# yupbank/tensorframes

Measured on AMD Instinct MI355X. Metric: rows/sec map_blocks MatMul on 10M-row DF at 1/2/4/8 MI355X, higher is better.
Workload: dtype fp32; 1 GPU; model=map_blocks relu(matmul(x[?,512], W[512,512])) float32, global_batch=10000000, seq_len=512, parallelism=dp1, partitions=4, rows=10000000

## Files before the change

csrc/bindings.cpp:

```cpp
#include <torch/extension.h>

#include <unordered_map>
#include <ATen/hip/HIPContext.h>
#include <c10/hip/HIPGuard.h>

#include "comm/comm.h"
#include "ir/graph.h"
#include "kernels/kernels.h"
#include "runtime/device_pool.h"
#include "runtime/executor.h"
#include "runtime/fusion.h"
#include "runtime/jit.h"
#include "runtime/jpeg_decode.h"
#include <rocprofiler-sdk-roctx/roctx.h>

namespace py = pybind11;
using namespace tfa;

namespace tfa {
void register_packer(py::module& m);
void register_pyencode(py::module& m);
}

namespace {

py::object shape_to_py(const Shape& s) {
  if (s.unknown_rank) return py::none();
  py::list l;
  for (auto d : s.dims) l.append(d);
  return l;
}

Shape shape_from_py(const py::object& o) {
  if (o.is_none()) return Shape::unknown();
  std::vector<int64_t> d;
  for (auto v : o) d.push_back(v.is_none() ? -1 : v.cast<int64_t>());
  return Shape(d);
}

const char* row_name(RowClass r) {
  switch (r) {
    case RowClass::CONST: return "const";
    case RowClass::ROW: return "row";
    default: return "mixed";
  }
}

std::map<std::string, TensorInfo> infos_from_py(const py::dict& d) {
  std::map<std::string, TensorInfo> m;
  for (auto kv : d) {
    auto t = kv.second.cast<py::tuple>();
    TensorInfo ti;
    ti.dtype = static_cast<DType>(t[0].cast<int>());
    ti.shape = shape_from_py(t[1]);
    m[kv.first.cast<std::string>()] = ti;
  }
  return m;
}

py::list infos_to_py(const std::vector<TensorInfo>& v) {
  py::list l;
  for (auto& ti : v) {
    py::dict d;
    d["dtype"] = static_cast<int>(ti.dtype);
    d["shape"] = shape_to_py(ti.shape);
    d["row"] = row_name(ti.row);
    d["const"] = ti.value.has_value();
    l.append(d);
  }
  return l;
}

py::dict infer_all(const std::string& bytes) {
  auto g = Graph::from_bytes(bytes);
  std::vector<TensorRef> all;
  for (size_t i = 0; i < g->nodes().size(); ++i) all.push_back({static_cast<int>(i), 0});
  auto order = g->closure(all);
  Graph::Infos infos = g->infer(order, {}, false);
  py::dict out;
  for (size_t i = 0; i < g->nodes().size(); ++i) out[py::str(g->node(i).name)] = infos_to_py(infos[i]);
  return out;
}

template <typename F, typename S>
at::Tensor key_image_typed(const at::Tensor& keys, at::ScalarType st) {
  at::Tensor out = pool_empty({keys.size(0)}, keys.options().dtype(st));
  const F* in = keys.data_ptr<F>();
  S* o = out.data_ptr<S>();
  const S flip = std::numeric_limits<S>::max();
  for (int64_t i = 0; i < keys.size(0); ++i) {
    F v = in[i];
    if (v != v) v = std::numeric_limits<F>::quiet_NaN();
    if (v == F(0)) v = F(0);
    S b;
    std::memcpy(&b, &v, sizeof(b));
    o[i] = b < 0 ? S(b ^ flip) : b;
  }
  return out;
}

template <typename F, typename S>
at::Tensor key_from_image_typed(const at::Tensor& img, at::ScalarType st) {
  at::Tensor out = pool_empty({img.size(0)}, img.options().dtype(st));
  const S* in = img.data_ptr<S>();
  F* o = out.data_ptr<F>();
  const S flip = std::numeric_limits<S>::max();
  for (int64_t i = 0; i < img.size(0); ++i) {
    S b = in[i] < 0 ? S(in[i] ^ flip) : in[i];
    std::memcpy(&o[i], &b, sizeof(b));
  }
  return out;
}

at::Tensor host_key_image(const at::Tensor& keys) {
  return keys.scalar_type() == at::kDouble ? key_image_typed<double, int64_t>(keys, at::kLong)
                                           : key_image_typed<float, int32_t>(keys, at::kInt);
}

at::Tensor host_key_from_image(const at::Tensor& img, at::ScalarType st) {
  return st == at::kDouble ? key_from_image_typed<double, int64_t>(img, st) : key_from_image_typed<float, int32_t>(img, st);
}

template <size_t N>
int name_index(const char* const (&names)[N], const std::string& s) {
  for (size_t i = 0; i < N; ++i)
    if (s == names[i]) return static_cast<int>(i);
  return -1;
}

void require_stat_type(at::ScalarType st, const std::string& subject, const char* object) {
  if (st != at::kFloat && st != at::kDouble && st != at::kLong && st != at::kInt && st != at::kShort &&
      st != at::kChar && st != at::kByte)
    throw py::type_error(str_cat(subject, c10::toString(st), object, ", which is not supported (uint8, int8, int16, "
                                 "int32, int64, float32 or float64)"));
}

void stat_column(const char* what, const at::Tensor& t, const std::string& which) {
  if (!t.is_cuda()) throw py::value_error(str_cat(what, ": ", which, " must be a device tensor"));
  if (t.dim() != 1) throw py::value_error(str_cat(what, ": ", which, " must be 1-D (one scalar per row)"));
  require_stat_type(t.scalar_type(), str_cat(what, ": ", which, " is "), "");
  if (!t.is_contiguous())
    throw py::value_error(str_cat(what, ": ", which, " is not contiguous; make it contiguous first"));
}

void stat_column_like(const char* what, const at::Tensor& t, const std::string& which, const char* ref,
                      const at::Device& dev, int64_t n, DType* dtype, const void** ptr) {
  stat_column(what, t, which);
  if (t.device() != dev) throw py::value_error(str_cat(what, ": ", which, " is not on ", ref, "'s device"));
  if (t.size(0) != n) throw py::value_error(str_cat(what, ": ", which, " has ", t.size(0), " rows, ", ref, " ", n));
  *dtype = from_scalar_type(t.scalar_type());
  *ptr = t.data_ptr();
}

k::StatCols stat_cols_from(const char* what, const std::vector<at::Tensor>& cols) {
  if (cols.empty() || cols.size() > static_cast<size_t>(k::kMaxPackCols))
    throw py::value_error(str_cat(what, ": 1..", k::kMaxPackCols, " columns per call, got ", cols.size()));
  k::StatCols sc;
  sc.n = static_cast<int>(cols.size());
  stat_column(what, cols[0], "column 0");
  for (size_t c = 0; c < cols.size(); ++c)
    stat_column_like(what, cols[c], str_cat("column ", c), "the first column", cols[0].device(), cols[0].size(0),
                     &sc.dtype[c], &sc.ptr[c]);
  return sc;
}

}

namespace tfa {
namespace k {
void set_conv_smallc(int on);
void set_conv_direct(int on);
}
void set_pool_conv_fusion(bool on);
}

static thread_local int g_sort_last_passes = 0;

PYBIND11_MODULE(TORCH_EXTENSION_NAME, m) {
  m.doc() = "tensorframes_amd native runtime (GraphDef executor + HIP/CDNA4 kernels)";

  py::register_exception<GraphError>(m, "GraphError", PyExc_ValueError);
  py::register_exception<comm::CollectiveError>(m, "CollectiveError", PyExc_RuntimeError);

  py::class_<Graph, std::shared_ptr<Graph>>(m, "Graph")
      .def(py::init([](py::bytes b) { return Graph::from_bytes(std::string(b)); }))
      .def("structure_key", [](const Graph& g) { return g.structure_key(); },
           "hash of the graph without its parameter constants' payloads (Graph::structure_key)")
      .def("parameter_consts",
           [](const Graph& g) {
             std::vector<std::string> v;
             const auto& p = g.parameter_consts();
             for (size_t i = 0; i < p.size(); ++i)
               if (p[i]) v.push_back(g.node(static_cast<int>(i)).name);
             return v;
           })
      .def("node_names",
           [](const Graph& g) {
             std::vector<std::string> v;
             for (auto& n : g.nodes()) v.push_back(n.name);
             return v;
           })
      .def("node_ops",
           [](const Graph& g) {
             std::vector<std::string> v;
             for (auto& n : g.nodes()) v.push_back(n.op);
             return v;
           })
      .def("node_inputs",
           [](const Graph& g, const std::string& name) {
             int i = g.find(name);
             TFA_CHECK(i >= 0, "no node named '", name, "'");
             return g.def().nodes[i].inputs;
           })
      .def("placeholders",
           [](const Graph& g) {
             std::vector<std::string> v;
             for (int i : g.placeholders()) v.push_back(g.node(i).name);
             return v;
           })
      .def("zero_input_nodes",
           [](const Graph& g) {
             std::vector<std::string> v;
             for (auto& n : g.nodes())
               if (n.inputs.empty() && n.control.empty()) v.push_back(n.name);
             return v;
           })
      .def("has_node", [](const Graph& g, const std::string& n) { return g.find(n) >= 0; })
      .def("node_attr_scalars",
           [](const Graph& g, const std::string& name) {
             int i = g.find(name);
             TFA_CHECK(i >= 0, "no node named '", name, "'");
             py::dict d;
             for (auto& kv : g.def().nodes[i].attr) {
               const AttrValue& a = kv.second;
               switch (a.kind) {
                 case AttrValue::I: d[py::str(kv.first)] = a.i; break;
                 case AttrValue::F: d[py::str(kv.first)] = a.f; break;
                 case AttrValue::B: d[py::str(kv.first)] = a.b; break;
                 case AttrValue::TYPE: d[py::str(kv.first)] = static_cast<int>(a.type); break;
                 case AttrValue::S: d[py::str(kv.first)] = py::bytes(a.s); break;
                 default: break;
               }
             }
             return d;
           })
      .def("const_strings",
           [](const Graph& g, const std::string& name) {
             int i = g.find(name);
             TFA_CHECK(i >= 0, "no node named '", name, "'");
             const NodeDef& nd = g.def().nodes[i];
             py::list l;
             const AttrValue* v = nd.find_attr("value");
             if (nd.op == "Const" && v && v->tensor && v->tensor->dtype == DType::STRING)
               for (auto& str : v->tensor->strings) l.append(py::bytes(str));
             return l;
           })
      .def("serialize", [](const Graph& g) { return py::bytes(serialize_graphdef(g.def())); })
      .def("__len__", [](const Graph& g) { return g.nodes().size(); });

  py::class_<Program, std::shared_ptr<Program>>(m, "Program")
      .def(py::init([](std::shared_ptr<Graph> g, std::vector<std::string> fetches,
                       std::vector<std::string> feeds) {
             return std::make_shared<Program>(g, fetches, feeds);
           }),
           py::arg("graph"), py::arg("fetches"), py::arg("feeds"))
      .def_property_readonly("fetch_names", &Program::fetch_names)
      .def_property_readonly("feed_names", &Program::feed_names)
      .def("row_separable",
           [](const Program& p, py::dict hints) { return p.row_separable(infos_from_py(hints)); })
      .def("rebind", &Program::rebind, py::arg("values"), py::call_guard<py::gil_scoped_release>(),
           "a program with new parameter-constant payloads that takes over this one's plans")
      .def("adopt", &Program::adopt, py::arg("old"), py::call_guard<py::gil_scoped_release>(),
           "take over the plans of a structurally equal program (see executor.h)")
      .def("monoids",
           [](const Program& p) {
             py::list l;
             for (auto& mi : p.monoids()) l.append(py::make_tuple(mi.fetch, mi.placeholder, mi.op));
             return l;
           })
      .def("run", &Program::run, py::call_guard<py::gil_scoped_release>())
      .def("run_concurrent", &Program::run_concurrent, py::arg("inputs_list"), py::arg("max_streams") = 4,
           py::call_guard<py::gil_scoped_release>(),
           "independent runs over several input sets on one GPU, forked onto engine side streams and joined "
           "back into the caller's stream")
      .def("run_chunked", &Program::run_chunked, py::arg("seg_inputs"), py::arg("seg_outputs"),
           py::arg("chunk_rows"), py::arg("device"), py::arg("depth") = 3, py::arg("wait") = true,
           py::call_guard<py::gil_scoped_release>())
      .def("release_pipeline", &Program::release_pipeline, py::call_guard<py::gil_scoped_release>(),
           "drain and free the persistent chunk pipeline (after a deferred run_chunked sequence)")
      .def("run_chunked_reduce", &Program::run_chunked_reduce, py::arg("seg_inputs"), py::arg("chunk_rows"),
           py::arg("device"), py::arg("depth") = 3, py::call_guard<py::gil_scoped_release>())
      .def("describe", &Program::describe_plan, py::arg("inputs"), py::arg("as_gpu") = false)
      .def("fused_sources", &Program::fused_sources)
      .def("reset_stats", &Program::reset_stats)
      .def("stats", [](const Program& p) {
        ExecStats s = p.stats();
        py::dict d;
        d["runs"] = s.runs;
        d["kernels"] = s.kernels;
        d["plans_built"] = s.plans_built;
        d["plans_adopted"] = s.plans_adopted;
        d["h2d_bytes"] = s.h2d_bytes;
        d["d2h_bytes"] = s.d2h_bytes;
        d["chunks"] = s.chunks;
        d["wall_ms"] = s.wall_ms;
        d["plan_ms"] = s.plan_ms;
        d["exec_ms"] = s.exec_ms;
        d["h2d_ms"] = s.h2d_ms;
        d["compute_ms"] = s.compute_ms;
        d["d2h_ms"] = s.d2h_ms;
        d["graphs_captured"] = s.graphs_captured;
        d["graph_replays"] = s.graph_replays;
        d["graph_failures"] = s.graph_failures;
        d["graphs_declined"] = s.graphs_declined;
        d["graph_busy"] = s.graph_busy;
        return d;
      });

  m.def("analyze_fetches",
        [](std::shared_ptr<Graph> g, std::vector<std::string> fetches, std::vector<std::string> feeds,
           py::dict hints) {
          Program p(g, fetches, feeds);
          Graph::Infos infos = p.analyze(infos_from_py(hints));
          py::dict out;
          auto info_of = [&](const std::string& f) -> py::object {
            TensorRef r = g->resolve(f);
            TFA_CHECK(r.index < static_cast<int>(infos[r.node].size()), "tensor '", f,
                      "' does not exist (node has ", infos[r.node].size(), " outputs)");
            py::list l = infos_to_py({infos[r.node][r.index]});
            return py::object(l[0]);
          };
          for (auto& f : fetches) out[py::str(f)] = info_of(f);
          for (auto& f : feeds) out[py::str(f)] = info_of(f);
          return out;
        });
  m.def("infer_fed",
        [](std::shared_ptr<Graph> g, std::vector<std::string> fetches, std::vector<std::string> feeds,
           py::dict hints) {
          Program p(g, fetches, feeds);
          Graph::Infos infos = p.analyze(infos_from_py(hints));
          py::dict out;
          for (size_t i = 0; i < infos.size(); ++i)
            if (!infos[i].empty()) out[py::str(g->node(static_cast<int>(i)).name)] = infos_to_py(infos[i]);
          return out;
        });
  m.def("infer_all", &infer_all);
  m.def("light_graphdef", [](py::bytes b, int64_t max_elems) {
    GraphDef g = parse_graphdef(std::string(b));
    for (auto& nd : g.nodes) {
      if (nd.op != "Const") continue;
      const AttrValue* v = nd.find_attr("value");
      if (!v || !v->tensor || v->tensor->num_elements() <= max_elems) continue;
      AttrValue dt;
      dt.kind = AttrValue::TYPE;
      dt.type = v->tensor->dtype;
      AttrValue shp;
      shp.kind = AttrValue::SHAPE;
      shp.shape = v->tensor->shape;
      nd.op = "Placeholder";
      nd.attr.clear();
      nd.attr["dtype"] = dt;
      nd.attr["shape"] = shp;
    }
    return py::bytes(serialize_graphdef(g));
  });
  m.def("patch_graphdef", [](py::bytes orig, py::bytes patch) {
    GraphDef g = parse_graphdef(std::string(orig));
    GraphDef p = parse_graphdef(std::string(patch));
    std::unordered_map<std::string, size_t> at;
    for (size_t i = 0; i < g.nodes.size(); ++i) at[g.nodes[i].name] = i;
    for (auto& nd : p.nodes) {
      auto it = at.find(nd.name);
      if (it != at.end()) g.nodes[it->second] = nd;
      else g.nodes.push_back(nd);
    }
    return py::bytes(serialize_graphdef(g));
  });
  m.def("registered_ops", [] { return OpRegistry::get().names(); });
  m.def("set_f32_precision", [](int mode) { k::set_f32_precision(mode); });
  m.def("factorize", [](const at::Tensor& keys0) {
    TFA_CHECK(keys0.dim() == 1, "factorize: keys must be 1-D");
    at::Tensor keys = keys0.contiguous();
    const int64_t n = keys.size(0);
    if (!keys.is_cuda()) {
      const bool fl = keys.scalar_type() == at::kFloat || keys.scalar_type() == at::kDouble;
      at::Tensor img = fl ? host_key_image(keys) : keys;
      auto r = at::_unique2(img, true, true, false);
      at::Tensor uniq = fl ? host_key_from_image(std::get<0>(r), keys.scalar_type()) : std::get<0>(r);
      return py::make_tuple(std::get<1>(r).to(at::kLong), uniq);
    }
    c10::hip::HIPGuard guard(keys.device().index());
    auto opts = keys.options();
    if (n == 0) return py::make_tuple(pool_empty({0}, opts.dtype(at::kLong)), pool_empty({0}, opts));
    hipStream_t s = c10::hip::getCurrentHIPStream(keys.device().index()).stream();
    const DType dt = from_scalar_type(keys.scalar_type());
    const size_t wsb = k::factorize_workspace_bytes(dt, n);
    at::Tensor ws = pool_empty({static_cast<int64_t>(wsb)}, opts.dtype(at::kByte));
    at::Tensor ids = pool_empty({n}, opts.dtype(at::kLong));
    at::Tensor uniq = pool_empty({n}, opts);
    int64_t nseg = 0;
    {
      py::gil_scoped_release nogil;
      nseg = k::factorize(dt, keys.data_ptr(), n, ids.data_ptr<int64_t>(), uniq.data_ptr(), ws.data_ptr(), wsb, s);
    }
    return py::make_tuple(ids, uniq.narrow(0, 0, nseg));
  }, "keys [n] -> (group id per row int64, distinct keys ascending)");
  m.def("string_words", [](const at::Tensor& offsets, const at::Tensor& data, int64_t W) {
    TFA_CHECK(offsets.scalar_type() == at::kLong && offsets.dim() == 1 && offsets.size(0) >= 1,
              "string_words: offsets must be int64[n+1]");
    TFA_CHECK(data.scalar_type() == at::kByte && data.dim() == 1, "string_words: data must be uint8[bytes]");
    TFA_CHECK(W >= 1 && W <= 4096, "string_words: 1..4096 words");
    TFA_CHECK(offsets.device() == data.device(), "string_words: offsets and data on different devices");
    const int64_t n = offsets.size(0) - 1;
    at::Tensor oc = offsets.contiguous(), dc = data.contiguous();
    if (!oc.is_cuda()) {
      at::Tensor out = at::empty({W + 1, n}, oc.options());
      const int64_t* o = oc.data_ptr<int64_t>();
      const uint8_t* d = dc.data_ptr<uint8_t>();
      int64_t* y = out.data_ptr<int64_t>();
      for (int64_t i = 0; i < n; ++i) {
        const int64_t a = o[i], len = o[i + 1] - a;
        for (int64_t w = 0; w < W; ++w) {
          uint64_t v = 0;
          for (int b = 0; b < 8; ++b) {
            const int64_t j = w * 8 + b;
            v |= static_cast<uint64_t>(j < len ? d[a + j] : 0) << (56 - 8 * b);
          }
          y[w * n + i] = static_cast<int64_t>(v ^ 0x8000000000000000ull);
        }
        y[W * n + i] = len;
      }
      return out;
    }
    c10::hip::HIPGuard guard(oc.device().index());
    at::Tensor out = pool_empty({W + 1, n}, oc.options());
    k::string_words(oc.data_ptr<int64_t>(), dc.data_ptr<uint8_t>(), n, static_cast<int>(W), out.data_ptr<int64_t>(),
                    c10::hip::getCurrentHIPStream(oc.device().index()).stream());
    return out;
  }, py::arg("offsets"), py::arg("data"), py::arg("words"),
        "string keys -> [words + 1, n] int64: big-endian 8-byte words (sign-flipped) + byte length; signed order "
        "of the columns = lexicographic order of the strings");
  m.def("string_key_hash", [](const at::Tensor& offsets, const at::Tensor& data) {
    TFA_CHECK(offsets.scalar_type() == at::kLong && offsets.dim() == 1 && offsets.size(0) >= 1,
              "string_key_hash: offsets must be int64[n+1]");
    TFA_CHECK(data.scalar_type() == at::kByte && data.dim() == 1, "string_key_hash: data must be uint8[bytes]");
    TFA_CHECK(offsets.device() == data.device(), "string_key_hash: offsets and data on different devices");
    const int64_t n = offsets.size(0) - 1;
    at::Tensor oc = offsets.contiguous(), dc = data.contiguous();
    if (!oc.is_cuda()) {
      at::Tensor out = at::empty({2, n}, oc.options());
      const int64_t* o = oc.data_ptr<int64_t>();
      const uint8_t* d = dc.data_ptr<uint8_t>();
      int64_t* y = out.data_ptr<int64_t>();
      for (int64_t i = 0; i < n; ++i) {
        const int64_t a = o[i], len = o[i + 1] - a;
        uint64_t v = 0;
        for (int b = 0; b < 8; ++b) v |= static_cast<uint64_t>(b < len ? d[a + b] : 0) << (56 - 8 * b);
        y[i] = static_cast<int64_t>(v ^ 0x8000000000000000ull);
        y[n + i] = len > 8 ? static_cast<int64_t>(k::string_key_hash_host(d + a, len) + 9) : len;
      }
      return out;
    }
    c10::hip::HIPGuard guard(oc.device().index());
    at::Tensor out = pool_empty({2, n}, oc.options());
    k::string_key_hash(oc.data_ptr<int64_t>(), dc.data_ptr<uint8_t>(), n, out.data_ptr<int64_t>(),
                   c10::hip::getCurrentHIPStream(oc.device().index()).stream());
    return out;
  }, py::arg("offsets"), py::arg("data"),
        "bounded-width string keys -> [2, n] int64: sign-flipped big-endian word 0, tag = length for keys of "
        "<= 8 bytes, else 9 + a 62-bit hash of the whole key");
  m.def("string_verify", [](const at::Tensor& offsets, const at::Tensor& data, const at::Tensor& ids,
                            const at::Tensor& rep) {
    TFA_CHECK(offsets.scalar_type() == at::kLong && ids.scalar_type() == at::kLong && rep.scalar_type() == at::kLong,
              "string_verify: int64 offsets / ids / representatives");
    const int64_t n = offsets.size(0) - 1;
    TFA_CHECK(ids.dim() == 1 && ids.size(0) == n, "string_verify: one id per string");
    TFA_CHECK(offsets.device() == data.device() && ids.device() == data.device() && rep.device() == data.device(),
              "string_verify: tensors on different devices");
    at::Tensor oc = offsets.contiguous(), dc = data.contiguous(), ic = ids.contiguous(), rc = rep.contiguous();
    if (!oc.is_cuda()) {
      const int64_t* o = oc.data_ptr<int64_t>();
      const uint8_t* d = dc.data_ptr<uint8_t>();
      const int64_t* id = ic.data_ptr<int64_t>();
      const int64_t* r = rc.data_ptr<int64_t>();
      for (int64_t i = 0; i < n; ++i) {
        const int64_t a = o[i], len = o[i + 1] - a, q = r[id[i]];
        if (len <= 8 || q == i) continue;
        if (o[q + 1] - o[q] != len || std::memcmp(d + a, d + o[q], len) != 0) return false;
      }
      return true;
    }
    c10::hip::HIPGuard guard(oc.device().index());
    hipStream_t st = c10::hip::getCurrentHIPStream(oc.device().index()).stream();
    at::Tensor flag = pool_empty({1}, oc.options().dtype(at::kInt));
    TFA_CHECK(hipMemsetAsync(flag.data_ptr(), 0, sizeof(int), st) == hipSuccess, "string_verify: memset failed");
    k::string_verify(oc.data_ptr<int64_t>(), dc.data_ptr<uint8_t>(), ic.data_ptr<int64_t>(), rc.data_ptr<int64_t>(), n,
                     flag.data_ptr<int>(), st);
    return flag.item<int>() == 0;
  }, "True when every string equals its group representative's (no hash collision)");
  m.def("gather_strings", [](const at::Tensor& offsets, const at::Tensor& data, const at::Tensor& idx) {
    TFA_CHECK(offsets.is_cuda() && data.is_cuda() && idx.is_cuda() && offsets.scalar_type() == at::kLong &&
                  idx.scalar_type() == at::kLong && data.scalar_type() == at::kByte,
              "gather_strings: device int64 offsets / idx and uint8 data expected");
    c10::hip::HIPGuard guard(data.device().index());
    hipStream_t st = c10::hip::getCurrentHIPStream(data.device().index()).stream();
    at::Tensor oc = offsets.contiguous(), ic = idx.contiguous(), dc = data.contiguous();
    const int64_t n = ic.numel();
    at::Tensor lens = pool_empty({std::max<int64_t>(n, 1)}, oc.options());
    k::string_lens(oc.data_ptr<int64_t>(), ic.data_ptr<int64_t>(), n, lens.data_ptr<int64_t>(), st);
    at::Tensor new_offs = at::empty({n + 1}, at::TensorOptions().dtype(at::kLong));
    int64_t* no = new_offs.data_ptr<int64_t>();
    no[0] = 0;
    if (n) {
      std::vector<int64_t> lh(n);
      TFA_CHECK(hipMemcpyAsync(lh.data(), lens.data_ptr(), n * sizeof(int64_t), hipMemcpyDeviceToHost, st) == hipSuccess &&
                    hipStreamSynchronize(st) == hipSuccess, "gather_strings: length copy failed");
      for (int64_t g = 0; g < n; ++g) no[g + 1] = no[g] + lh[g];
    }
    at::Tensor out = pool_empty({std::max<int64_t>(no[n], 1)}, dc.options());
    if (n) {
      at::Tensor dno = pool_empty({n + 1}, oc.options());
      TFA_CHECK(hipMemcpyAsync(dno.data_ptr(), no, (n + 1) * sizeof(int64_t), hipMemcpyHostToDevice, st) == hipSuccess,
                "gather_strings: offset copy failed");
      k::gather_bytes(dc.data_ptr<uint8_t>(), oc.data_ptr<int64_t>(), ic.data_ptr<int64_t>(), dno.data_ptr<int64_t>(), n,
                      out.data_ptr<uint8_t>(), st);
      TFA_CHECK(hipStreamSynchronize(st) == hipSuccess, "gather_strings: gather failed");
    }
    return py::make_tuple(new_offs, out.narrow(0, 0, no[n]));
  }, "rows idx of a device string column -> (host int64 offsets [n+1], device uint8 bytes)");
  m.def("key_dest", [](const std::vector<at::Tensor>& keys, int64_t world) {
    TFA_CHECK(!keys.empty() && keys[0].is_cuda(), "key_dest: device key columns expected");
    c10::hip::HIPGuard guard(keys[0].device().index());
    const int64_t n = keys[0].size(0);
    hipStream_t s = c10::hip::getCurrentHIPStream(keys[0].device().index()).stream();
    at::Tensor h = pool_empty({n}, keys[0].options().dtype(at::kLong));
    for (size_t i = 0; i < keys.size(); ++i) {
      at::Tensor kc = keys[i].contiguous();
      TFA_CHECK(kc.dim() == 1 && kc.size(0) == n, "key_dest: key columns must be 1-D of equal length");
      k::key_hash(from_scalar_type(kc.scalar_type()), kc.data_ptr(), n,
                  reinterpret_cast<uint64_t*>(h.data_ptr<int64_t>()), i > 0, s);
    }
    at::Tensor dest = pool_empty({n}, h.options());
    k::hash_mod(reinterpret_cast<const uint64_t*>(h.data_ptr<int64_t>()), n, world, dest.data_ptr<int64_t>(), s);
    return dest;
  }, "destination rank of every row: hash(keys) % world (same on every rank)");
  m.def("group_representatives", [](const at::Tensor& ids, int64_t nseg) {
    TFA_CHECK(ids.is_cuda() && ids.scalar_type() == at::kLong && ids.dim() == 1, "group_representatives: device int64 ids");
    c10::hip::HIPGuard guard(ids.device().index());
    at::Tensor rep = pool_empty({nseg}, ids.options());
    k::group_representatives(ids.contiguous().data_ptr<int64_t>(), ids.size(0), nseg, rep.data_ptr<int64_t>(),
                             c10::hip::getCurrentHIPStream(ids.device().index()).stream());
    return rep;
  }, "the last row index of every group (device), as the host path's rep[ids] = arange(n)");
  m.def("partition_rows", [](const at::Tensor& dest0, int64_t world) {
    TFA_CHECK(dest0.is_cuda() && dest0.scalar_type() == at::kLong && dest0.dim() == 1, "partition_rows: device int64 dest");
    c10::hip::HIPGuard guard(dest0.device().index());
    at::Tensor dest = dest0.contiguous();
    const int64_t n = dest.size(0);
    hipStream_t s = c10::hip::getCurrentHIPStream(dest.device().index()).stream();
    const size_t wsb = k::partition_workspace_bytes(n);
    at::Tensor ws = pool_empty({static_cast<int64_t>(wsb)}, dest.options().dtype(at::kByte));
    at::Tensor perm = pool_empty({n}, dest.options());
    at::Tensor counts = pool_empty({world}, dest.options());
    k::partition_rows(dest.data_ptr<int64_t>(), n, world, perm.data_ptr<int64_t>(), counts.data_ptr<int64_t>(),
                      ws.data_ptr(), wsb, s);
    return py::make_tuple(perm, counts);
  }, "rows ordered by destination rank (stable) + rows per destination (device)");
  m.def("segment_csr", [](const at::Tensor& ids0, int64_t nseg) {
    TFA_CHECK(ids0.is_cuda() && ids0.dim() == 1 && (ids0.scalar_type() == at::kLong || ids0.scalar_type() == at::kInt),
              "segment_csr: device int ids");
    c10::hip::HIPGuard guard(ids0.device().index());
    at::Tensor ids = ids0.contiguous();
    const int64_t n = ids.size(0);
    hipStream_t s = c10::hip::getCurrentHIPStream(ids.device().index()).stream();
    at::Tensor perm = pool_empty({n}, ids.options().dtype(at::kLong));
    at::Tensor off = pool_empty({nseg + 1}, ids.options().dtype(at::kLong));
    const size_t wsb = k::segment_csr_workspace_bytes(n, nseg);
    at::Tensor ws = pool_empty({static_cast<int64_t>(wsb)}, ids.options().dtype(at::kByte));
    k::segment_csr(from_scalar_type(ids.scalar_type()), ids.data_ptr(), n, nseg, perm.data_ptr<int64_t>(),
                   off.data_ptr<int64_t>(), ws.data_ptr(), wsb, s);
    return py::make_tuple(perm, off);
  }, "ids [n] in [0, nseg) -> (rows ordered by segment, stable; CSR offsets [nseg + 1]) on the device");
  m.def("segment_rows", [](const at::Tensor& perm, const at::Tensor& offs, int64_t size) {
    TFA_CHECK(perm.is_cuda() && offs.is_cuda() && perm.scalar_type() == at::kLong && offs.scalar_type() == at::kLong,
              "segment_rows: device int64 tensors");
    c10::hip::HIPGuard guard(perm.device().index());
    const int64_t G = offs.size(0);
    at::Tensor idx = pool_empty({G * size}, perm.options());
    k::segment_rows(perm.contiguous().data_ptr<int64_t>(), offs.contiguous().data_ptr<int64_t>(), G, size,
                    idx.data_ptr<int64_t>(), c10::hip::getCurrentHIPStream(perm.device().index()).stream());
    return idx;
  }, "row ids of G equal-size segments: perm[offs[g] + j] for j < size -> [G * size]");
  m.def("scatter_rows", [](at::Tensor dst, const at::Tensor& idx, const at::Tensor& src0) {
    TFA_CHECK(dst.is_cuda() && idx.is_cuda() && src0.is_cuda() && idx.scalar_type() == at::kLong,
              "scatter_rows: device tensors");
    TFA_CHECK(dst.is_contiguous() && dst.dim() >= 1 && src0.scalar_type() == dst.scalar_type(),
              "scatter_rows: contiguous dst of the source dtype");
    c10::hip::HIPGuard guard(dst.device().index());
    at::Tensor src = src0.contiguous();
    TFA_CHECK(src.size(0) == idx.size(0), "scatter_rows: one index per source row");
    const int64_t row = dst.size(0) ? dst.numel() / dst.size(0) : 0;
    TFA_CHECK(src.numel() == idx.size(0) * row, "scatter_rows: source rows must match the destination row shape");
    k::scatter_rows(row * dst.element_size(), src.data_ptr(), idx.contiguous().data_ptr<int64_t>(), dst.data_ptr(),
                    idx.size(0), c10::hip::getCurrentHIPStream(dst.device().index()).stream());
    return dst;
  }, "dst[idx[j]] = src[j] along dim 0 (device scatter kernel), in place");
  m.def("pack_rows", [](const std::vector<at::Tensor>& cols, std::optional<at::Tensor> perm) {
// ... 1206 lines not shown
    if (!x.is_cuda()) {
      int64_t cols = 1;
      for (int64_t i = 1; i < x.dim(); ++i) cols *= x.size(i);
      at::Tensor il = ids.to(at::kLong);
      at::Tensor valid = (il >= 0) & (il < nseg);
      at::Tensor xs = x.reshape({nrows, cols}).index({valid});
      at::Tensor is = il.index({valid});
      at::Tensor out;
      if (rop == k::RedOp::SUM) {
        out = at::zeros({nseg, cols}, x.options()).index_add_(0, is, xs);
      } else if (rop == k::RedOp::PROD) {
        out = at::ones({nseg, cols}, x.options()).index_reduce_(0, is, xs, "prod", true);
      } else {
        const bool mx = rop == k::RedOp::MAX;
        at::Scalar init;
        bool known = true;
        switch (x.scalar_type()) {
          case at::kInt: init = mx ? std::numeric_limits<int32_t>::lowest() : std::numeric_limits<int32_t>::max(); break;
          case at::kLong: init = mx ? std::numeric_limits<int64_t>::lowest() : std::numeric_limits<int64_t>::max(); break;
          case at::kFloat: init = mx ? std::numeric_limits<float>::lowest() : std::numeric_limits<float>::max(); break;
          case at::kDouble: init = mx ? std::numeric_limits<double>::lowest() : std::numeric_limits<double>::max(); break;
          default: known = false;
        }
        out = known ? at::full({nseg, cols}, init, x.options()) : at::empty({nseg, cols}, x.options());
        out = out.index_reduce_(0, is, xs, mx ? "amax" : "amin", known);
      }
      out = out.reshape(osz).contiguous();
      if (out_opt) return out_opt->copy_(out);
      return out;
    }
    c10::hip::HIPGuard guard(x.device().index());
    at::Tensor xc = x.contiguous(), ic = ids.contiguous();
    at::Tensor out;
    if (out_opt) {
      out = *out_opt;
      TFA_CHECK(out.is_cuda() && out.is_contiguous() && out.sizes().vec() == osz && out.scalar_type() == xc.scalar_type(),
                "unsorted_segment_reduce: out must be a contiguous device tensor of the result shape and dtype");
    } else {
      out = pool_empty(osz, xc.options());
    }
    if (!out.numel()) return out;
    const int64_t inner = out.numel() / nseg;
    const DType dt = from_scalar_type(xc.scalar_type());
    size_t ws = k::unsorted_segment_workspace_bytes(rop, dt, nrows, inner, nseg);
    at::Tensor work;
    if (ws) work = pool_empty({static_cast<int64_t>(ws)}, xc.options().dtype(at::kByte));
    k::unsorted_segment_reduce(rop, dt, from_scalar_type(ic.scalar_type()), xc.data_ptr(), ic.data_ptr(),
                               out.data_ptr(), nrows, inner, nseg, ws ? work.data_ptr() : nullptr,
                               c10::hip::getCurrentHIPStream(x.device().index()).stream());
    return out;
  }, py::arg("op"), py::arg("x"), py::arg("ids"), py::arg("nseg"), py::arg("out") = py::none());
  m.def("segment_reduce", [](const std::string& op, const at::Tensor& x, const at::Tensor& offsets) {
    TFA_CHECK(x.dim() >= 1, "segment_reduce needs rank >= 1");
    TFA_CHECK(offsets.scalar_type() == at::kLong && offsets.dim() == 1, "offsets must be int64[nseg+1]");
    int64_t nseg = offsets.size(0) - 1;
    std::vector<int64_t> osz = x.sizes().vec();
    osz[0] = nseg;
    k::RedOp rop = op == "Sum" ? k::RedOp::SUM : op == "Min" ? k::RedOp::MIN : op == "Max" ? k::RedOp::MAX
                 : op == "Prod" ? k::RedOp::PROD : op == "Mean" ? k::RedOp::MEAN : k::RedOp::ALL;
    TFA_CHECK(rop != k::RedOp::ALL, "segment_reduce: unsupported op ", op);
    if (!x.is_cuda()) {
      at::Tensor off = offsets.to(at::kCPU);
      const int64_t* o = off.data_ptr<int64_t>();
      std::vector<at::Tensor> parts;
      for (int64_t s = 0; s < nseg; ++s) {
        at::Tensor seg = x.narrow(0, o[s], o[s + 1] - o[s]);
        switch (rop) {
          case k::RedOp::SUM: parts.push_back(seg.sum(0, false, x.scalar_type())); break;
          case k::RedOp::MIN: parts.push_back(std::get<0>(seg.min(0))); break;
          case k::RedOp::MAX: parts.push_back(std::get<0>(seg.max(0))); break;
          case k::RedOp::PROD: parts.push_back(seg.prod(0, false, x.scalar_type())); break;
          default: parts.push_back(seg.to(at::kDouble).mean(0).to(x.scalar_type()));
        }
      }
      return nseg ? at::stack(parts, 0) : at::empty(osz, x.options());
    }
    c10::hip::HIPGuard guard(x.device().index());
    at::Tensor xc = x.contiguous();
    at::Tensor out = pool_empty(osz, xc.options());
    int64_t inner = nseg ? out.numel() / nseg : 0;
    if (out.numel())
      k::segment_reduce_csr(rop, from_scalar_type(xc.scalar_type()), xc.data_ptr(),
                            offsets.contiguous().data_ptr<int64_t>(), out.data_ptr(), nseg, inner,
                            c10::hip::getCurrentHIPStream(x.device().index()).stream());
    return out;
  });
  m.def("empty_pinned", &empty_pinned);
  m.def("trim_pinned_pool", &trim_pinned_pool);
  m.def("is_pinned", [](const at::Tensor& t) {
    if (t.is_cuda() || !t.numel()) return false;
    hipPointerAttribute_t attr;
    if (hipPointerGetAttributes(&attr, t.data_ptr()) != hipSuccess) {
      (void)hipGetLastError();
      return false;
    }
    return attr.type == hipMemoryTypeHost;
  });
  m.def("pinned_pool_cached_bytes", &pinned_pool_cached_bytes);
  m.def("device_pool_stats", [] {
    DevPoolStats v = dev_pool_stats();
    py::dict d;
    d["allocs"] = v.allocs;
    d["frees"] = v.frees;
    d["fallbacks"] = v.fallbacks;
    d["capture_allocs"] = v.capture_allocs;
    d["device_mallocs"] = v.device_mallocs;
    d["live"] = v.live_bytes;
    d["peak"] = v.peak_bytes;
    d["cached"] = v.cached_bytes;
    return d;
  }, "engine-owned device pool: allocations, frees, c10 fallbacks, HIP-graph capture allocations, hipMallocs, live / peak / cached bytes");
  m.def("trim_device_pool", &dev_pool_trim);
  {
    using comm::Comm;
    using GR = py::call_guard<py::gil_scoped_release>;
    py::class_<Comm, std::shared_ptr<Comm>>(m, "Comm",
        "engine communicator: all_reduce / all_gather / all_to_all_v / broadcast on the current stream")
        .def_property_readonly("rank", &Comm::rank)
        .def_property_readonly("size", &Comm::size)
        .def_property_readonly("kind", &Comm::kind)
        .def_property_readonly("calls", &Comm::calls)
        .def("all_reduce", [](Comm& c, at::Tensor t, const std::string& op) {
          c.all_reduce(t, comm::parse_op(op));
          return t;
        }, py::arg("tensor"), py::arg("op") = "Sum", GR())
        .def("all_gather", &Comm::all_gather, GR())
        .def("all_to_all_v", &Comm::all_to_all_v, py::arg("x"), py::arg("send_rows"), py::arg("recv_rows"), GR())
        .def("broadcast", [](Comm& c, at::Tensor t, int root) {
          c.broadcast(t, root);
          return t;
        }, py::arg("tensor"), py::arg("root") = 0, GR())
        .def("barrier", &Comm::barrier, GR());
    py::class_<comm::FakeWorld, std::shared_ptr<comm::FakeWorld>>(m, "FakeWorld",
        "N in-process ranks over host memory (CPU test double of the communicator)")
        .def(py::init<int>())
        .def_property_readonly("size", &comm::FakeWorld::size)
        .def("comm", [](std::shared_ptr<comm::FakeWorld> w, int r) {
          return std::shared_ptr<Comm>(std::make_shared<comm::FakeComm>(w, r));
        });
    py::class_<comm::RcclComm, Comm, std::shared_ptr<comm::RcclComm>>(m, "RcclComm",
        "an RCCL communicator of the engine's own (ncclCommInitRank)")
        .def(py::init([](py::bytes uid, int rank, int size, int device) {
          std::string u = uid;
          py::gil_scoped_release nogil;
          return std::make_shared<comm::RcclComm>(u, rank, size, device);
        }), py::arg("unique_id"), py::arg("rank"), py::arg("size"), py::arg("device"))
        .def("abort", &comm::RcclComm::abort, GR())
        .def("async_error", &comm::RcclComm::async_error)
        .def("set_timeout", &comm::RcclComm::set_timeout, py::arg("seconds"), py::arg("exit_on_timeout") = true,
             "seconds a collective may take (<= 0: unbounded); past it wait() raises CollectiveError, and past it "
             "plus a grace period the watchdog thread aborts the communicator and exits the process "
             "(exit_on_timeout) or marks it failed")
        .def_property_readonly("timeout", &comm::RcclComm::timeout)
        .def("wait", &comm::RcclComm::wait, GR(), "bounded wait for every collective issued so far")
        .def("check", &comm::RcclComm::check, "raises CollectiveError if the communicator failed")
        .def_property_readonly("failed", &comm::RcclComm::failed)
        .def_property_readonly("inflight", &comm::RcclComm::inflight)
        .def("set_test_stall", &comm::RcclComm::set_test_stall, py::arg("seconds"),
             "tests: a spin kernel inside each all_reduce, after its start event");
    py::class_<comm::ShmComm, Comm, std::shared_ptr<comm::ShmComm>>(m, "ShmComm",
        "host tensors of the ranks of one node through a POSIX shared-memory segment")
        .def(py::init<const std::string&, int, int, int64_t, bool>(), py::arg("name"), py::arg("rank"),
             py::arg("size"), py::arg("slot_bytes"), py::arg("create"), GR())
        .def("unlink", &comm::ShmComm::unlink)
        .def("set_timeout", &comm::ShmComm::set_timeout, py::arg("seconds"))
        .def("poison", &comm::ShmComm::poison, "make every rank's current / next collective raise")
        .def("reset_after_failure", &comm::ShmComm::reset_after_failure,
             "clear the barrier state (only once every rank has left the communicator)")
        .def_property_readonly("poisoned", &comm::ShmComm::poisoned)
        .def_property_readonly("slot_bytes", &comm::ShmComm::slot_bytes)
        .def_property_readonly("attached", &comm::ShmComm::attached);
    m.attr("EXIT_COLLECTIVE_TIMEOUT") = comm::kExitCollectiveTimeout;
    m.def("device_stall", [](double seconds) {
      k::device_stall(static_cast<uint64_t>(std::max(0.0, seconds) * 1e6),
                      c10::hip::getCurrentHIPStream().stream());
    }, py::arg("seconds"), "fault injection: a bounded (<= 60 s) spin kernel on the current stream");
    m.def("can_access_peer", [](int a, int b) {
      int ok = 0;
      if (hipDeviceCanAccessPeer(&ok, a, b) != hipSuccess) {
        (void)hipGetLastError();
        return false;
      }
      return ok != 0;
    }, py::arg("device"), py::arg("peer"));
    m.def("rccl_unique_id", [] { return py::bytes(comm::rccl_unique_id()); });
    py::class_<comm::OneShotComm, std::shared_ptr<comm::OneShotComm>>(m, "OneShotComm",
        "single-hop all-reduce of payloads <= 64 KB through IPC-mapped peer buffers")
        .def(py::init<int, int, int>(), py::arg("rank"), py::arg("size"), py::arg("device"))
        .def("ipc_handle", [](comm::OneShotComm& o) { return py::bytes(o.ipc_handle()); })
        .def("open", &comm::OneShotComm::open)
        .def_property_readonly("ready", &comm::OneShotComm::ready)
        .def_property_readonly("calls", &comm::OneShotComm::calls)
        .def_static("max_bytes", &comm::OneShotComm::max_bytes)
        .def("all_reduce", [](comm::OneShotComm& o, at::Tensor t, const std::string& op) {
          o.all_reduce(t, comm::parse_op(op));
          return t;
        }, py::arg("tensor"), py::arg("op") = "Sum", GR())
        .def("check", &comm::OneShotComm::check, GR())
        .def("set_timeout", &comm::OneShotComm::set_timeout, py::arg("seconds"))
        .def_property_readonly("alloc_kind", &comm::OneShotComm::alloc_kind)
        .def_property_readonly("failed", &comm::OneShotComm::failed);
  }
  m.def("cat_rows", [](const std::vector<at::Tensor>& ts) {
    TFA_CHECK(!ts.empty(), "cat_rows: no tensors");
    const at::Tensor& t0 = ts[0];
    TFA_CHECK(t0.is_cuda() && t0.dim() >= 1, "cat_rows: device tensors of rank >= 1 expected");
    std::vector<int64_t> sz = t0.sizes().vec();
    int64_t rows = 0;
    for (auto& t : ts) {
      TFA_CHECK(t.is_cuda() && t.device() == t0.device() && t.scalar_type() == t0.scalar_type() &&
                    t.dim() == t0.dim() && t.sizes().slice(1) == t0.sizes().slice(1),
                "cat_rows: tensors must share device, dtype and trailing shape");
      rows += t.size(0);
    }
    sz[0] = rows;
    c10::hip::HIPGuard guard(t0.device().index());
    at::Tensor out = pool_empty(sz, t0.options());
    hipStream_t st = c10::hip::getCurrentHIPStream(t0.device().index()).stream();
    std::vector<at::Tensor> keep;
    k::CopyPieces pc;
    int64_t off = 0;
    auto flush = [&]() {
      k::batched_copy(pc, out.data_ptr(), st);
      pc.n = 0;
    };
    for (auto& t0i : ts) {
      at::Tensor t = t0i.is_contiguous() ? t0i : t0i.contiguous();
      if (!t0i.is_contiguous()) keep.push_back(t);
      const int64_t nb = t.numel() * t.element_size();
      if (nb) {
        pc.src[pc.n] = t.data_ptr();
        pc.dst_off[pc.n] = off;
        pc.bytes[pc.n] = nb;
        if (++pc.n == k::kMaxCopyPieces) flush();
      }
      off += nb;
    }
    flush();
    for (auto& t : keep) dev_record_stream(t, st);
    return out;
  }, py::arg("tensors"), "row concatenation of device tensors into one pool buffer: one batched-copy kernel");
  m.def("cat_rows_many", [](const std::vector<std::vector<at::Tensor>>& cols) {
    TFA_CHECK(!cols.empty() && !cols[0].empty(), "cat_rows_many: no tensors");
    const at::Tensor& t00 = cols[0][0];
    TFA_CHECK(t00.is_cuda(), "cat_rows_many: device tensors expected");
    std::vector<std::vector<int64_t>> shapes;
    std::vector<int64_t> offs;
    int64_t total = 0;
    for (auto& ts : cols) {
      TFA_CHECK(!ts.empty(), "cat_rows_many: empty column");
      const at::Tensor& t0 = ts[0];
      TFA_CHECK(t0.dim() >= 1, "cat_rows_many: tensors of rank >= 1 expected");
      std::vector<int64_t> sz = t0.sizes().vec();
      int64_t rows = 0, nb = 0;
      for (auto& t : ts) {
        TFA_CHECK(t.is_cuda() && t.device() == t00.device() && t.scalar_type() == t0.scalar_type() &&
                      t.dim() == t0.dim() && t.sizes().slice(1) == t0.sizes().slice(1),
                  "cat_rows_many: the tensors of a column must share device, dtype and trailing shape");
        rows += t.size(0);
        nb += t.numel() * t.element_size();
      }
      sz[0] = rows;
      shapes.push_back(sz);
      offs.push_back(total);
      total += (nb + 255) / 256 * 256;
    }
    c10::hip::HIPGuard guard(t00.device().index());
    at::Tensor buf = pool_empty({std::max<int64_t>(total, 1)}, t00.options().dtype(at::kByte));
    hipStream_t st = c10::hip::getCurrentHIPStream(t00.device().index()).stream();
    std::vector<at::Tensor> keep;
    k::CopyPieces pc;
    auto flush = [&]() {
      k::batched_copy(pc, buf.data_ptr(), st);
      pc.n = 0;
    };
    for (size_t c = 0; c < cols.size(); ++c) {
      int64_t off = offs[c];
      for (auto& t0i : cols[c]) {
        at::Tensor t = t0i.is_contiguous() ? t0i : t0i.contiguous();
        if (!t0i.is_contiguous()) keep.push_back(t);
        const int64_t nb = t.numel() * t.element_size();
        if (nb) {
          pc.src[pc.n] = t.data_ptr();
          pc.dst_off[pc.n] = off;
          pc.bytes[pc.n] = nb;
          if (++pc.n == k::kMaxCopyPieces) flush();
        }
        off += nb;
      }
    }
    flush();
    for (auto& t : keep) dev_record_stream(t, st);
    std::vector<at::Tensor> out;
    for (size_t c = 0; c < cols.size(); ++c) {
      const auto dt = cols[c][0].scalar_type();
      int64_t n = 1;
      for (int64_t d : shapes[c]) n *= d;
      out.push_back(buf.narrow(0, offs[c], n * c10::elementSize(dt)).view(dt).view(shapes[c]));
    }
    return out;
  }, py::arg("columns"), "row concatenations of several columns into one pool buffer (views of it)");
  m.def("pipeline_wait", &pipeline_wait, py::arg("handle"), py::call_guard<py::gil_scoped_release>(),
        "wait for a run_chunked(wait=False) completion handle (and release it)");
  m.def("device_empty", [](const std::vector<int64_t>& sizes, at::ScalarType dt, int device) {
    c10::hip::HIPGuard guard(static_cast<c10::DeviceIndex>(device));
    return pool_empty(sizes, at::TensorOptions().dtype(dt).device(at::kCUDA, static_cast<c10::DeviceIndex>(device)));
  }, py::arg("sizes"), py::arg("dtype"), py::arg("device"),
        "uninitialised device tensor from the engine pool, ordered on the device's current stream");
  m.def("device_zeros", [](const std::vector<int64_t>& sizes, at::ScalarType dt, int device) {
    c10::hip::HIPGuard guard(static_cast<c10::DeviceIndex>(device));
    return pool_zeros(sizes, at::TensorOptions().dtype(dt).device(at::kCUDA, static_cast<c10::DeviceIndex>(device)));
  }, py::arg("sizes"), py::arg("dtype"), py::arg("device"), "zeroed (hipMemsetAsync) device tensor from the engine pool");
  m.def("fill_", [](at::Tensor& t, double value) {
    TFA_CHECK(t.is_cuda() && t.is_contiguous(), "fill_: contiguous device tensor expected");
    c10::hip::HIPGuard guard(t.device().index());
    k::fill(from_scalar_type(t.scalar_type()), t.data_ptr(), t.numel(), value,
            c10::hip::getCurrentHIPStream(t.device().index()).stream());
    return t;
  }, py::arg("tensor"), py::arg("value"), "fill a device tensor in place (kernels/elementwise fill)");
  m.def("record_stream", [](const at::Tensor& t, uint64_t stream) {
    TFA_CHECK(t.is_cuda(), "record_stream: device tensor expected");
    dev_record_stream(t, reinterpret_cast<hipStream_t>(stream));
  }, py::arg("tensor"), py::arg("stream"),
        "the tensor is also used on `stream` (a hipStream_t handle): its memory (engine pool or c10) is not "
        "reused before that stream's work queued so far has finished");
  m.def("pinned_pool_stats", [] {
    auto v = pinned_pool_stats();
    py::dict d;
    d["limit"] = v[0];
    d["cached"] = v[1];
    d["live"] = v[2];
    d["peak"] = v[3];
    return d;
  }, "page-locked pool: cap, cached free bytes, live bytes, peak live bytes");
  m.def("pin_host_tensor", &pin_host_tensor);
  m.def("unpin_host_tensor", &unpin_host_tensor);
}
```

csrc/kernels/kernels.h:

```cpp
#pragma once

#include <hip/hip_runtime.h>

#include <cstdint>
#include <utility>
#include <vector>

#include "../common.h"

namespace tfa {
namespace k {

constexpr int kMaxRank = 8;

void check_launch(const char* what);

enum class BinOp : int {
  ADD, SUB, MUL, DIV, FLOORDIV, FLOORMOD, TRUNCMOD, MAX, MIN, POW, SQDIFF,
  EQ, NE, LT, LE, GT, GE, LAND, LOR, ATAN2, DIVNONAN,
};
enum class UnOp : int {
  NEG, ABS, SQUARE, SQRT, RSQRT, EXP, LOG, LOG1P, EXPM1, RECIP, RELU, RELU6, ELU, SELU,
  SIGMOID, TANH, SOFTPLUS, SOFTSIGN, FLOOR, CEIL, ROUND, SIGN, SIN, COS, TAN, NOT, IDENTITY,
  ERF, ISNAN, ISINF, ISFINITE,
};

struct Bcast {
  int rank = 0;
  int64_t dims[kMaxRank];
  int64_t sa[kMaxRank];
  int64_t sb[kMaxRank];
  int64_t sc[kMaxRank];
};

void binary(BinOp op, DType dt, const void* a, const void* b, void* out, int64_t n, int mode,
            int64_t inner, const Bcast* bc, hipStream_t s);
void unary(UnOp op, DType dt, const void* x, void* y, int64_t n, hipStream_t s);
void cast(DType from, DType to, const void* x, void* y, int64_t n, hipStream_t s);
void select(DType dt, const void* cond, const void* a, const void* b, void* out, int64_t n,
            const Bcast& bc, hipStream_t s);
void fill(DType dt, void* out, int64_t n, double value, hipStream_t s);
void range(DType dt, void* out, int64_t n, double start, double delta, hipStream_t s);


enum class RedOp : int { SUM, PROD, MIN, MAX, MEAN, ALL, ANY };
size_t reduce_workspace_bytes(DType dt, int64_t outer, int64_t r, int64_t inner);
void reduce(RedOp op, DType dt, const void* x, void* y, int64_t outer, int64_t r, int64_t inner,
            void* workspace, hipStream_t s);
enum class RedRoute : int {
  ROW_WAVE_VEC, ROW_WAVE, ROW_BLOCK, ROW_SPLIT, ROW_SPLIT_FOLD,
  COL, COL_VEC, COL_SPLIT, COL_VEC_SPLIT, COL_SPLIT_FOLD, COL_VEC_SPLIT_FOLD, COUNT
};
struct ReducePlan {
  RedRoute route;
  int64_t S = 1;
  int64_t rows_per_split = 0;
  int64_t fold = 0;
  int64_t col_blocks = 0;
  int vec = 1;
};
const char* reduce_route_name(RedRoute r);
ReducePlan reduce_route(DType dt, int64_t outer, int64_t r, int64_t inner, bool aligned16);
void argreduce(bool is_min, DType dt, DType out_dt, const void* x, void* y, int64_t outer,
               int64_t r, int64_t inner, hipStream_t s);
void softmax(DType dt, bool log, const void* x, void* y, int64_t rows, int64_t cols, hipStream_t s);
void topk(DType dt, const void* x, void* vals, int32_t* idx, int64_t rows, int64_t cols, int k,
          hipStream_t s);
constexpr int kOneShotMaxRanks = 8;
constexpr size_t kOneShotSlotBytes = 64 << 10;
constexpr size_t kOneShotFlagOffset = 2 * kOneShotSlotBytes;
constexpr size_t kOneShotErrOffset = kOneShotFlagOffset + 2 * 8 * 4;
constexpr size_t kOneShotBufBytes = kOneShotErrOffset + 256;
struct OneShotPeers {
  void* buf[kOneShotMaxRanks];
};
void oneshot_all_reduce(RedOp op, DType dt, const void* in, void* out, int64_t n, int rank, int world,
                        const OneShotPeers& p, uint32_t epoch, uint64_t timeout_us, hipStream_t s);
void device_stall(uint64_t us, hipStream_t s);

size_t unsorted_segment_workspace_bytes(RedOp op, DType dt, int64_t n, int64_t inner, int64_t nseg);
void unsorted_segment_reduce(RedOp op, DType dt, DType idt, const void* x, const void* ids,
                             void* y, int64_t n, int64_t inner, int64_t nseg, void* workspace,
                             hipStream_t s);
enum class UsegRoute : int { TINY_INT, SMALL_INT, PRIVATE, SORTED_PERM };
struct UsegPlan {
  UsegRoute route;
  int64_t B = 0;
  int G = 0;
  int64_t tile = 0;
  int64_t rows_per_block = 0;
  int inner_pad = 0;
  bool wide = false;
};
UsegPlan unsorted_segment_route(RedOp op, DType dt, int64_t n, int64_t inner, int64_t nseg);
std::string unsorted_segment_route_name(const UsegPlan& p);
void segment_reduce_csr(RedOp op, DType dt, const void* x, const int64_t* offsets, void* y,
                        int64_t nseg, int64_t inner, hipStream_t s);

size_t factorize_workspace_bytes(DType dt, int64_t n);
int64_t factorize(DType dt, const void* keys, int64_t n, int64_t* ids, void* uniq, void* workspace,
                  size_t workspace_size, hipStream_t s);
void key_hash(DType dt, const void* keys, int64_t n, uint64_t* h, bool accumulate, hipStream_t s);
void hash_mod(const uint64_t* h, int64_t n, int64_t world, int64_t* dest, hipStream_t s);
void string_words(const int64_t* offs, const uint8_t* data, int64_t n, int W, int64_t* out, hipStream_t s);
void string_key_hash(const int64_t* offs, const uint8_t* data, int64_t n, int64_t* out, hipStream_t s);
void string_verify(const int64_t* offs, const uint8_t* data, const int64_t* ids, const int64_t* rep, int64_t n,
                   int* flag, hipStream_t s);
uint64_t string_key_hash_host(const uint8_t* p, int64_t len);
void string_lens(const int64_t* offs, const int64_t* idx, int64_t n, int64_t* lens, hipStream_t s);
void gather_bytes(const uint8_t* data, const int64_t* offs, const int64_t* idx, const int64_t* new_offs, int64_t n,
                  uint8_t* out, hipStream_t s);
size_t segment_csr_workspace_bytes(int64_t n, int64_t nseg);
void segment_csr(DType idt, const void* ids, int64_t n, int64_t nseg, int64_t* perm, int64_t* offsets,
                 void* workspace, size_t workspace_size, hipStream_t s);
void segment_reduce_perm(RedOp op, DType dt, const void* x, const int64_t* perm, const int64_t* offsets, void* y,
                         int64_t nseg, int64_t inner, hipStream_t s);
void group_representatives(const int64_t* ids, int64_t n, int64_t nseg, int64_t* rep, hipStream_t s);
void segment_rows(const int64_t* perm, const int64_t* offs, int64_t G, int64_t size, int64_t* idx, hipStream_t s);
void scatter_rows(int64_t row_bytes, const void* src, const int64_t* idx, void* dst, int64_t nidx, hipStream_t s);
constexpr int kMaxPackCols = 16;
struct PackCols {
  int n = 0;
  int64_t row_bytes[kMaxPackCols];
  int64_t off[kMaxPackCols];
  const void* ptr[kMaxPackCols];
};
void pack_rows(const PackCols& pc, const int64_t* perm, int64_t nrows, int64_t record_bytes, void* out,
               hipStream_t s);
void unpack_rows(const PackCols& pc, const void* in, int64_t nrows, int64_t record_bytes, hipStream_t s);
size_t partition_workspace_bytes(int64_t n);
void partition_rows(const int64_t* dest, int64_t n, int64_t world, int64_t* perm, int64_t* counts, void* workspace,
                    size_t workspace_size, hipStream_t s);

int compact_tile_rows();
size_t compact_workspace_bytes(int64_t n);
int64_t compact_plan(const uint8_t* mask, int64_t n, void* workspace, size_t workspace_size, hipStream_t s);
void compact_gather(const PackCols& src, const PackCols& dst, const uint8_t* mask, int64_t n, int64_t total,
                    const void* workspace, int64_t* index, hipStream_t s);

constexpr int kMaxSortKeys = 8;
struct SortKeys {
  int n = 0;
  DType dtype[kMaxSortKeys];
  const void* ptr[kMaxSortKeys];
  int descending[kMaxSortKeys];
};
void sort_encode(const SortKeys& keys, int64_t n, int64_t* words, hipStream_t s);
int sort_tile_rows();
size_t sort_argsort_workspace_bytes(int W, int64_t n);
int sort_argsort(const int64_t* words, int W, int64_t n, int64_t* perm, void* workspace, size_t workspace_size,
                 hipStream_t s);
void permute_rows(const PackCols& src, const PackCols& dst, const int64_t* perm, int64_t n, hipStream_t s);
void take_rows(const PackCols& src, const PackCols& dst, const int64_t* idx, int64_t n_out, int64_t n_src,
               hipStream_t s);
void sort_bounds(const int64_t* words, int W, int64_t n, const int64_t* perm, const int64_t* splitters, int64_t S,
                 int64_t* out, hipStream_t s);

void join_gather_words(const int64_t* words, int W, int64_t m, const int64_t* perm, int64_t* out, hipStream_t s);
void join_probe(const int64_t* left, int W, int64_t n, const int64_t* right_sorted, int64_t m, int64_t* lo,
                int64_t* cnt, uint8_t* mask, int mask_mode, hipStream_t s);
size_t join_scan_workspace_bytes(int64_t n);
int64_t join_scan(const int64_t* cnt, int64_t n, int64_t m, int64_t* offs, void* workspace, size_t workspace_size,
                  hipStream_t s);
int join_tile_rows();
void join_expand(const int64_t* offs, const int64_t* lo, const int64_t* perm, int64_t n, int64_t m, int64_t total,
                 int64_t* left_idx, int64_t* right_idx, hipStream_t s);

struct StatCols {
  int n = 0;
  DType dtype[kMaxPackCols];
  const void* ptr[kMaxPackCols];
};
size_t column_moments_workspace_bytes(int ncols, int64_t n);
void column_moments(const StatCols& cols, int64_t n, double* moments, int64_t* extremes, void* workspace,
                    size_t workspace_size, hipStream_t s);
constexpr int kPairRecordFields = 7;
size_t column_pair_moments_workspace_bytes(int npairs, int64_t n);
void column_pair_moments(const StatCols& xs, const StatCols& ys, int64_t n, int64_t* records, void* workspace,
                         size_t workspace_size, hipStream_t s);
int stats_tile_rows();
void select_hist(DType dtype, const void* col, int64_t n, const int64_t* prefixes, int P, int prefix_bits,
                 int64_t* hist, hipStream_t s);

constexpr int kGroupRecordFields = 6;
int group_chunk_rows();
struct GroupItems {
  const int64_t* coffs = nullptr;
  int64_t items = 0;
};
size_t group_items_workspace_bytes(int64_t nseg);
GroupItems group_items(const int64_t* offsets, int64_t nseg, int64_t nperm, void* workspace, size_t workspace_size,
                       hipStream_t s);
size_t group_moments_workspace_bytes(int ncols, int64_t nperm, int64_t nseg);
void group_moments(const StatCols& cols, int64_t n, const int64_t* perm, int64_t nperm, const int64_t* offsets,
                   int64_t nseg, int64_t* records, void* workspace, size_t workspace_size, hipStream_t s,
                   const GroupItems* items = nullptr);
size_t group_pair_moments_workspace_bytes(int npairs, int64_t nperm, int64_t nseg);
void group_pair_moments(const StatCols& xs, const StatCols& ys, int64_t n, const int64_t* perm, int64_t nperm,
                        const int64_t* offsets, int64_t nseg, int64_t* records, void* workspace, size_t workspace_size,
                        hipStream_t s, const GroupItems* items = nullptr);
void merge_group_records(const int64_t* records, int64_t m, int ncols, uint32_t float_mask, const int64_t* offsets,
                         int64_t ng, int64_t* out, hipStream_t s);
enum class GroupStat : int { COUNT = 0, SUM, AVG, MIN, MAX, VAR_SAMP, VAR_POP, STDDEV_SAMP, STDDEV_POP };
struct GroupResultSpec {
  int n = 0;
  int col[kMaxPackCols];
  GroupStat stat[kMaxPackCols];
  DType dtype[kMaxPackCols];
  void* out[kMaxPackCols];
};
void group_results(const int64_t* records, int64_t ng, int ncols, const GroupResultSpec& spec, hipStream_t s);
void merge_pair_records(const int64_t* records, int64_t m, int npairs, const int64_t* offsets, int64_t ng,
                        int64_t* out, hipStream_t s);
enum class PairStat : int { CORR = 0, COVAR_SAMP, COVAR_POP };
struct PairResultSpec {
  int n = 0;
  int pair[kMaxPackCols];
  PairStat stat[kMaxPackCols];
  double* out[kMaxPackCols];
};
void pair_results(const int64_t* records, int64_t ng, int npairs, const PairResultSpec& spec, hipStream_t s);

enum class WindowChan : int { GROUP_HEAD = 0, PEER_HEAD, PEER_COUNT, SUM_I64, SUM_F64, MIN_WORD, MAX_WORD };
struct WindowChans {
  int n = 0;
  int kind[kMaxPackCols];
  DType dtype[kMaxPackCols];
  const void* ptr[kMaxPackCols];
};
int window_tile_rows();
int window_chan_op(int kind);
size_t window_scan_workspace_bytes(int nchan, int64_t n);
void window_scan(const int64_t* words, int W, int P, int64_t n, bool reverse, const WindowChans& ch, int64_t* out,
                 void* workspace, size_t workspace_size, hipStream_t s);
enum class WindowFn : int { ROW_NUMBER = 0, RANK, DENSE_RANK, COUNT, SUM, AVG, MIN, MAX };
enum class WindowFrame : int { ROWS = 0, RANGE, WHOLE };
struct WindowFinishSpec {
  int n_out = 0;
  WindowFn fn[kMaxPackCols];
  WindowFrame frame[kMaxPackCols];
  int chan[kMaxPackCols];
  DType dtype[kMaxPackCols];
  void* out[kMaxPackCols];
  int n_chan = 0;
  int op[kMaxPackCols];
  uint64_t carry[kMaxPackCols];
  uint64_t total[kMaxPackCols];
  int has_carry = 0, has_total = 0;
  int64_t carry_rows = 0, total_rows = 0;
};
void window_finish(const int64_t* fwd, const int64_t* rev, int64_t n, const WindowFinishSpec& spec, hipStream_t s);

constexpr int kMaxCopyPieces = 32;
struct CopyPieces {
  const void* src[kMaxCopyPieces];
  int64_t dst_off[kMaxCopyPieces];
  int64_t bytes[kMaxCopyPieces];
  int n = 0;
};
void batched_copy(const CopyPieces& pc, void* dst, hipStream_t s);
void strided_copy(int64_t elem_size, int rank, const int64_t* dims, const void* src,
                  const int64_t* src_strides, void* dst, const int64_t* dst_strides,
                  hipStream_t s);
void gather(int64_t elem_size, DType idt, const void* params, const void* idx, void* out,
            int64_t outer, int64_t axis_dim, int64_t nidx, int64_t inner, hipStream_t s);
void one_hot(DType dt, DType idt, const void* idx, void* out, int64_t n, int64_t depth,
             double on, double off, hipStream_t s);

enum Act : int { ACT_NONE = 0, ACT_RELU = 1, ACT_RELU6 = 2, ACT_SIGMOID = 3, ACT_TANH = 4, ACT_ELU = 5,
                 ACT_SELU = 6, ACT_SOFTPLUS = 7 };

enum EpiCode : int { EPI_ADD = 0, EPI_SUB, EPI_RSUB, EPI_MUL, EPI_DIV, EPI_RDIV, EPI_MAX, EPI_MIN, EPI_ACT, EPI_NEG,
                     EPI_SQUARE, EPI_ABS };
enum EpiOperand : int { EPO_NONE = 0, EPO_SCALAR, EPO_SCALAR_PTR, EPO_COL, EPO_ROW, EPO_FULL };
struct EpiOp {
  int code = EPI_ADD, kind = EPO_NONE, act = ACT_NONE;
  double s = 0;
  const void* p = nullptr;
};
constexpr int kMaxEpi = 6;
struct EpiProg {
  int n = 0;
  EpiOp op[kMaxEpi];
};

constexpr int kMaxOutSegs = 4;
struct OutSegs {
  int n = 0;
  int64_t begin[kMaxOutSegs + 1];
  void* ptr[kMaxOutSegs];
  int64_t ldc[kMaxOutSegs];
  int act[kMaxOutSegs];
};

struct GemmArgs {
  int64_t M, N, K;
  const void* A; int64_t lda; int64_t strideA;
  const void* B; int64_t ldb; int64_t strideB;
  void* C; int64_t ldc; int64_t strideC;
  bool ta, tb;
  const void* bias;
  int act;
  int64_t batch;
  void* workspace = nullptr;
  EpiProg epi;
  OutSegs seg;
};
size_t gemm_workspace_bytes(DType dt, const GemmArgs& g);
void gemm(DType dt, const GemmArgs& g, hipStream_t s);
void set_f32_precision(int mode);
void set_gemm_tile(int cfg);
int gemm_tile_count();
std::vector<std::pair<std::vector<int64_t>, int>> gemm_tune_table();
void gemm_tune_seed(const std::vector<int64_t>& key, int cfg);
void gemm_tune_reset();
std::vector<int> gemm_tile_dims(int cfg);
int f32_precision();
enum class F64Tile : int { T64x16, T64x64, T128x128, COUNT };
constexpr int64_t kGemmMaxBatchPerLaunch = 65535;
struct GemmF64Plan {
  F64Tile tile;
  int BM, BN;
  int64_t tiles_m, tiles_n;
  int64_t launches;
  bool k_mult16;
  bool a_pairs, b_pairs;
};
const char* gemm_f64_tile_name(F64Tile t);
GemmF64Plan gemm_f64_route(int64_t M, int64_t N, int64_t K, int64_t batch, bool ta, bool tb, int64_t lda,
                           int64_t ldb, bool a_aligned16, bool b_aligned16);
struct GemmIntPlan {
  int64_t tiles_m, tiles_n;
  int64_t launches;
};
GemmIntPlan gemm_int_route(int64_t M, int64_t N, int64_t K, int64_t batch);

struct ConvArgs {
  int64_t N, H, W, C;
  int64_t KH, KW, OC;
  int64_t OH, OW;
  int64_t sh, sw, dh, dw;
  int64_t pad_t, pad_l;
  const void* x; const void* w; void* y;
  const void* bias; int act;
  void* workspace = nullptr;
  int64_t ldc = 0;
  EpiProg epi;
  OutSegs seg;
  const void* wino = nullptr;
  bool pool2 = false;
};
size_t conv2d_workspace_bytes(DType dt, const ConvArgs& a);
void conv2d_nhwc(DType dt, const ConvArgs& a, hipStream_t s);
bool conv2d_pool2_direct(const ConvArgs& a);
const char* last_conv_algo();
void set_last_conv_algo(const char* label);
const char* last_f32_tile();
struct PoolArgs {
  int64_t N, H, W, C, OH, OW, KH, KW, sh, sw, pad_t, pad_l;
  bool is_max;
  const void* x; void* y;
  const void* bias = nullptr;
  int act = 0;
  int64_t ldc = 0;
};
void pool2d_nhwc(DType dt, const PoolArgs& a, hipStream_t s);
enum class PoolRoute : int {
  P3X3_V4_XCD, P3X3_V4, GENERIC_V4_U32, GENERIC_V4_I64, GENERIC_V1_U32, GENERIC_V1_I64, COUNT
};
struct PoolPlan {
  PoolRoute route;
  int V;
  int64_t items;
  int64_t blocks;
};
const char* pool_route_name(PoolRoute r);
PoolPlan pool_route(const PoolArgs& a, bool x_aligned16, bool y_aligned16);
void set_pool_route(int route);
struct PoolConvArgs {
  int64_t N, H, W, C, PH, PW, pkh, pkw, psh, psw, OC, ldc;
  const void* x; const void* w; const void* bias; void* y;
  int act = 0;
};
bool pool_conv1x1_eligible(int64_t N, int64_t H, int64_t W, int64_t C, int64_t PH, int64_t PW, int64_t OC,
                           int64_t ldc, int act);
void pool_conv1x1(const PoolConvArgs& a, hipStream_t s);
int conv_wino_kind(int64_t KH, int64_t KW, int64_t sh, int64_t sw, int64_t dh, int64_t dw, int64_t C, int64_t OC);
int64_t conv_wino_ocp(int64_t OC);
int64_t conv_wino_filter_elems(int kind, int64_t C, int64_t OC);
void conv_wino_filter(int kind, const float* w, int64_t C, int64_t OC, float* u);
void set_conv_wino(int on);
bool conv_wino_enabled();
void set_wino_tile(int v);
void set_wino_bn(int bn);
void set_wino_5x5(int on);
struct ResizeArgs {
  int64_t N, H, W, C, OH, OW;
  float sh, sw;
  int mode;
  const void* x; void* y;
};
void resize_bilinear(DType dt, const ResizeArgs& a, hipStream_t s);
void resize_nearest(int64_t elem_size, const ResizeArgs& a, hipStream_t s);
struct RaggedPrepArgs {
  int64_t n = 0;
  int C = 3, OH = 0, OW = 0, oy = 0, ox = 0, h = 0, w = 0, mode = 0;
  int nops = 0;
  int op_kind[4] = {0, 0, 0, 0}, op_chan[4] = {0, 0, 0, 0};
  float op_val[4][4] = {};
  const uint8_t* x = nullptr;
  const int64_t* offs = nullptr;
  const int32_t* hw = nullptr;
  const int32_t* rp = nullptr;
  float* y = nullptr;
};
void ragged_image_prep(const RaggedPrepArgs& a, hipStream_t s);
struct PadArgs {
  int rank = 0, mode = 0;
  int64_t out_dims[kMaxRank], in_dims[kMaxRank], in_strides[kMaxRank], before[kMaxRank];
};
void pad_nd(int64_t elem_size, const PadArgs& a, const void* x, void* y, uint64_t cbits, hipStream_t s);
void scan(bool prod, DType dt, const void* x, void* y, int64_t outer, int64_t n, int64_t inner, bool exclusive,
          bool reverse, hipStream_t s);
void leaky_relu(DType dt, const void* x, void* y, int64_t n, double alpha, hipStream_t s);
struct DepthwiseArgs {
  int64_t N, H, W, C, M, KH, KW, OH, OW, sh, sw, dh, dw, pad_t, pad_l;
  const void* x; const void* w; void* y;
};
void depthwise_conv2d_nhwc(const DepthwiseArgs& a, hipStream_t s);
void lrn(DType dt, const void* x, void* y, int64_t n, int64_t C, int radius, double bias, double alpha, double beta,
         hipStream_t s);
struct GatherNdArgs {
  int K = 0;
  int64_t dims[kMaxRank], strides[kMaxRank];
};
void gather_nd(int64_t elem_size, DType idt, const void* params, const void* idx, void* out, int64_t nidx,
               int64_t inner, const GatherNdArgs& a, hipStream_t s);
struct WhereArgs {
  int rank = 0;
  int64_t dims[kMaxRank];
};
void mask_prefix(const uint8_t* mask, int64_t* pos, int64_t n, hipStream_t s);
// ... 9 lines not shown
```

csrc/runtime/executor.cpp:

```cpp
#include "executor.h"

#include <optional>
#include "device_pool.h"


#include <ATen/hip/HIPContext.h>
#include <c10/hip/HIPCachingAllocator.h>
#include <c10/hip/HIPGuard.h>
#include <hip/hip_runtime.h>
#include <rocprofiler-sdk-roctx/roctx.h>

#include <algorithm>
#include <array>
#include <atomic>
#include <chrono>
#include <unistd.h>
#include <cstdlib>
#include <set>
#include <unordered_map>
#include <sstream>

#include "../ir/ops_common.h"
#include "fusion.h"
#include "hip_graph.h"
#include "jit.h"

namespace tfa {


namespace {

#define HIP_OK(expr)                                                                  \
  do {                                                                                \
    hipError_t _e = (expr);                                                           \
    TFA_CHECK(_e == hipSuccess, "HIP error ", hipGetErrorString(_e), " at ", #expr); \
  } while (0)

std::atomic<int> g_debug_sync{-1};

bool debug_sync() {
  int v = g_debug_sync.load(std::memory_order_relaxed);
  if (v < 0) {
    const char* e = std::getenv("TFA_DEBUG_SYNC");
    int want = (e && e[0] == '1') ? 1 : 0;
    g_debug_sync.compare_exchange_strong(v, want);
    v = g_debug_sync.load(std::memory_order_relaxed);
  }
  return v == 1;
}

struct RangeGuard {
  explicit RangeGuard(const std::string& name) { roctxRangePushA(name.c_str()); }
  ~RangeGuard() { roctxRangePop(); }
};

std::atomic<bool> g_step_timing{false};
struct StepRec {
  std::string node, op, label;
  double flops = 0, bytes = 0;
  hipEvent_t a = nullptr, b = nullptr;
};
std::mutex g_step_mu;
std::vector<StepRec> g_step_recs;

bool stage_timers_enabled() {
  static const bool on = [] {
    const char* e = std::getenv("TFA_STAGE_TIMERS");
    return !(e && e[0] == '0');
  }();
  return on;
}

int epilogue_act(const std::string& op) {
  static const std::map<std::string, int> m = {
      {"Relu", k::ACT_RELU},   {"Relu6", k::ACT_RELU6}, {"Sigmoid", k::ACT_SIGMOID}, {"Tanh", k::ACT_TANH},
      {"Elu", k::ACT_ELU},     {"Selu", k::ACT_SELU},   {"Softplus", k::ACT_SOFTPLUS}};
  auto it = m.find(op);
  return it == m.end() ? k::ACT_NONE : it->second;
}

const char* act_name(int act) {
  static const char* names[] = {"none", "relu", "relu6", "sigmoid", "tanh", "elu", "selu", "softplus"};
  return act >= 0 && act < 8 ? names[act] : "?";
}

bool epi_chain_enabled() {
  static const bool on = [] {
    const char* e = std::getenv("TFA_EPI_CHAIN");
    return !(e && e[0] == '0');
  }();
  return on;
}

bool sibling_fusion_enabled() {
  static const bool on = [] {
    const char* e = std::getenv("TFA_SIBLING_FUSION");
    return !(e && e[0] == '0');
  }();
  return on;
}

bool pool_fusion_enabled() {
  static const bool on = [] {
    const char* e = std::getenv("TFA_POOL_FUSION");
    return !(e && e[0] == '0');
  }();
  return on;
}

int pipe_compute_streams() {
  static const int n = [] {
    const char* e = std::getenv("TFA_PIPE_COMPUTE_STREAMS");
    return e && e[0] == '1' ? 1 : 2;
  }();
  return n;
}

std::atomic<int>& pool_conv_fusion_state() {
  static std::atomic<int> v([] {
    const char* e = std::getenv("TFA_POOL_CONV_FUSION");
    return (e && e[0] == '0') ? 0 : 1;
  }());
  return v;
}

}

void set_pool_conv_fusion(bool on) { pool_conv_fusion_state().store(on ? 1 : 0); }

namespace {

bool conv_pool_fusion_enabled() {
  static const bool on = [] {
    const char* e = std::getenv("TFA_CONV_POOL_FUSION");
    return !(e && e[0] == '0');
  }();
  return on;
}

bool gemm_ta(const Node& nd) {
  return nd.op == "MatMul" ? nd.attr_b("transpose_a", false) : nd.attr_b("adj_x", false);
}
bool gemm_tb(const Node& nd) {
  return nd.op == "MatMul" ? nd.attr_b("transpose_b", false) : nd.attr_b("adj_y", false);
}

std::string strip0(const std::string& s) {
  if (s.size() > 2 && s.compare(s.size() - 2, 2, ":0") == 0) return s.substr(0, s.size() - 2);
  return s;
}

}

void set_debug_sync(bool on) { g_debug_sync.store(on ? 1 : 0); }

hipStream_t copy_stream(int device, int which) {
  static std::mutex mu;
  static std::map<std::pair<int, int>, hipStream_t> streams;
  std::lock_guard<std::mutex> lk(mu);
  auto it = streams.find({device, which});
  if (it != streams.end()) return it->second;
  int cur = 0;
  TFA_CHECK(hipGetDevice(&cur) == hipSuccess, "hipGetDevice failed");
  TFA_CHECK(hipSetDevice(device) == hipSuccess, "hipSetDevice failed");
  hipStream_t st = nullptr;
  hipError_t e = hipStreamCreateWithFlags(&st, hipStreamNonBlocking);
  (void)hipSetDevice(cur);
  TFA_CHECK(e == hipSuccess, "hipStreamCreate failed: ", hipGetErrorString(e));
  streams[{device, which}] = st;
  return st;
}
bool get_debug_sync() { return debug_sync(); }

struct Program::Step {
  enum Kind { OP, GEMM, CONV, FUSED } kind = OP;
  int fused = -1;
  int node = -1;
  int out_node = -1;
  std::vector<int> in_slots;
  std::vector<int> out_slots;
  std::vector<TensorInfo> out_info;
  std::vector<const TensorInfo*> in_info;
  int bias_slot = -1;
  TensorRef bias_ref{-1, 0};
  int act = 0;
  struct Epi {
    int code, kind, act;
    double s;
    int slot;
    TensorRef ref;
  };
  std::vector<Epi> epi;
  Shape gemm_shape;
  std::vector<int> release;
  int alias_slot = -1;
  int64_t alias_offset = 0;
  const TensorInfo* alias_info = nullptr;
  std::vector<char> preplaced;
  struct Sib {
    int node;
    int64_t oc;
    int alias_slot;
    int64_t alias_offset;
    const TensorInfo* alias_info;
    int act;
  };
  std::vector<Sib> sibs;
  int wino_slot = -1;
  bool pool2 = false;
  int pool_in[4] = {0, 0, 0, 0};
};

struct Program::Plan {
  Graph::Infos infos;
  std::vector<Step> steps;
  int nslots = 0;
  std::vector<int> feed_slots;
  std::vector<std::pair<int, TensorRef>> const_slots;
  std::map<int, at::Tensor> synth_consts;
  std::vector<int> fetch_slots;
  std::map<int, std::map<int, at::Tensor>> dev_consts;
  std::map<int, TensorInfo> feed_infos;
  std::shared_ptr<Graph> base_graph;
  struct Arena {
    at::Tensor dev;
    std::vector<std::tuple<int, TensorRef, size_t, size_t>> items;
  };
  std::map<int, Arena> arenas;
  std::set<int> stale;
  bool cap_reset = false;
  std::map<int, void*> last_stream;
  std::map<int, std::set<void*>> used_streams;
  int fused = 0;
  int fused_siblings = 0;
  int wino_convs = 0;
  struct Fused {
    FusedRegion region;
    std::mutex mu;
    std::map<int, jit::Kernel> kernels;
  };
  std::vector<std::unique_ptr<Fused>> fused_regions;
  struct ReplayOrder {
    hipStream_t last = nullptr;
    void before(hipStream_t cur) {
      if (last && last != cur) (void)hipStreamSynchronize(last);
    }
    void after(hipStream_t cur) { last = cur; }
    void drain() {
      if (last) (void)hipStreamSynchronize(last);
      last = nullptr;
    }
  };
  struct Captured {
    std::mutex mu;
    int64_t gpu_runs = 0;
    bool failed = false;
    int64_t eager_ns = 0, eager_n = 0, replay_ns = 0, replay_n = 0;
    bool declined = false;
    int device = -1;
    hipStream_t stream = nullptr;
    std::unique_ptr<HipGraph> graph;
    std::vector<at::Tensor> static_in, static_out;
    ReplayOrder order;
    ~Captured() {
      order.drain();
      graph.reset();
      if (stream) (void)hipStreamDestroy(stream);
    }
  } cap;
  struct PtrCap : AliasUseSink {
    bool cloning = false;
    std::unique_ptr<HipGraph> graph;
    std::vector<at::Tensor> static_out;
    std::vector<long> base_uc;
    std::vector<bool> input_alias;
    hipStream_t stream = nullptr;
    int64_t last_use = 0;
    ReplayOrder order;
    std::mutex use_mu;
    std::vector<hipEvent_t> uses;
    bool outputs_free() const {
      for (size_t i = 0; i < static_out.size(); ++i)
        if (!input_alias[i] && static_out[i].storage().use_count() > base_uc[i]) return false;
      return true;
    }
    void record_use(hipStream_t s) override {
      hipEvent_t e;
      if (hipEventCreateWithFlags(&e, hipEventDisableTiming) != hipSuccess) {
        (void)hipGetLastError();
        (void)hipStreamSynchronize(s);
        return;
      }
      (void)hipEventRecord(e, s);
      std::lock_guard<std::mutex> lk(use_mu);
      uses.push_back(e);
    }
    void wait_uses(hipStream_t cur) {
      std::lock_guard<std::mutex> lk(use_mu);
      for (hipEvent_t e : uses) {
        (void)hipStreamWaitEvent(cur, e, 0);
        (void)hipEventDestroy(e);
      }
      uses.clear();
    }
    ~PtrCap() override;
  };
  std::mutex ptr_mu;
  std::map<std::vector<const void*>, int> ptr_seen;
  std::map<std::vector<const void*>, std::vector<std::unique_ptr<PtrCap>>> ptr_caps;
  int64_t ptr_tick = 0;
  bool ptr_declined = false;
  int64_t ptr_eager_ns = 0, ptr_eager_n = 0, ptr_replay_ns = 0, ptr_replay_n = 0;
};

namespace {
std::mutex g_alias_mu;
std::unordered_map<const void*, Program::AliasUseSink*>& alias_registry() {
  static auto* m = new std::unordered_map<const void*, Program::AliasUseSink*>();
  return *m;
}
void register_aliases(Program::AliasUseSink* sink, const std::vector<const void*>& ptrs) {
  std::lock_guard<std::mutex> lk(g_alias_mu);
  for (const void* q : ptrs) alias_registry()[q] = sink;
}
void unregister_aliases(Program::AliasUseSink* sink, const std::vector<const void*>& ptrs) {
  std::lock_guard<std::mutex> lk(g_alias_mu);
  for (const void* q : ptrs) {
    auto it = alias_registry().find(q);
// ... 1495 lines not shown
    }
    c.graph = std::move(g);
    stats_.graphs_captured++;
  }
  c.order.before(cur);
  for (size_t i = 0; i < inputs.size(); ++i) c.static_in[i].copy_(inputs[i], true);
  wait_consts(inputs[0].device(), cur);
  {
    std::lock_guard<std::mutex> cl(const_mu_);
    p.used_streams[dev].insert(cur);
  }
  c.graph->replay(cur);
  std::vector<at::Tensor> outs = clone_outputs(c.static_out, cur);
  c.order.after(cur);
  stats_.graph_replays++;
  return outs;
}

namespace {
constexpr int kPtrWarmRuns = 2;
constexpr size_t kPtrMinSteps = 3;
constexpr size_t kPtrMaxCaps = 8;
constexpr size_t kPtrMaxSeen = 32;
int64_t ptr_graph_max_bytes() {
  static const int64_t v = env_positive("TFA_HIP_GRAPH_PTR_MAX_BYTES", int64_t(256) << 20);
  return v;
}
}

std::optional<std::vector<at::Tensor>> Program::run_ptr_graph(Plan& p, const std::vector<at::Tensor>& inputs,
                                                               int64_t bytes) {
  if (hip_graphs_mode() != 1 || p.ptr_declined || p.cap_reset || bytes > ptr_graph_max_bytes() ||
      p.steps.size() < kPtrMinSteps || inputs.empty())
    return std::nullopt;
  for (auto& t : inputs)
    if (!t.is_cuda() || !t.is_contiguous()) return std::nullopt;
  std::vector<const void*> key;
  key.reserve(inputs.size());
  for (auto& t : inputs) key.push_back(t.data_ptr());
  std::lock_guard<std::mutex> lk(p.ptr_mu);
  const int dev = inputs[0].device().index();
  hipStream_t cur = c10::hip::getCurrentHIPStream(dev).stream();
  auto it = p.ptr_caps.find(key);
  Plan::PtrCap* use = nullptr;
  if (it != p.ptr_caps.end()) {
    for (auto& c : it->second)
      if (!c->cloning && c->outputs_free()) use = c.get();
    if (!use)
      for (auto& c : it->second)
        if (c->cloning) use = c.get();
  }
  const bool cloning = it != p.ptr_caps.end() && (use ? use->cloning : true);
  if (!use) {
    if (it == p.ptr_caps.end()) {
      int& seen = p.ptr_seen[key];
      if (p.ptr_seen.size() > kPtrMaxSeen) {
        p.ptr_seen.clear();
        return std::nullopt;
      }
      if (++seen <= kPtrWarmRuns || !graphable(p)) {
        if (seen > 1) {
          const int64_t t0 = now_ns();
          auto outs = execute(p, inputs, cur);
          p.ptr_eager_ns += now_ns() - t0;
          p.ptr_eager_n++;
          return outs;
        }
        return std::nullopt;
      }
    }
    size_t total = 0;
    for (auto& kv : p.ptr_caps) total += kv.second.size();
    if (total >= kPtrMaxCaps) {
      std::vector<std::unique_ptr<Plan::PtrCap>>* lv = nullptr;
      size_t li = 0;
      int64_t best = INT64_MAX;
      for (auto& kv : p.ptr_caps)
        for (size_t i = 0; i < kv.second.size(); ++i)
          if (kv.second[i]->last_use < best) {
            best = kv.second[i]->last_use;
            lv = &kv.second;
            li = i;
          }
      if (lv) {
        auto& victim = (*lv)[li];
        if (victim->stream) (void)hipStreamSynchronize(victim->stream);
        victim->order.drain();
        lv->erase(lv->begin() + static_cast<long>(li));
        for (auto j = p.ptr_caps.begin(); j != p.ptr_caps.end();)
          j = j->second.empty() ? p.ptr_caps.erase(j) : std::next(j);
      }
    }
    auto pc = std::make_unique<Plan::PtrCap>();
    TFA_CHECK(hipStreamCreateWithFlags(&pc->stream, hipStreamNonBlocking) == hipSuccess, "hipStreamCreate failed");
    hipEvent_t ev;
    TFA_CHECK(hipEventCreateWithFlags(&ev, hipEventDisableTiming) == hipSuccess, "hipEventCreate failed");
    (void)hipEventRecord(ev, cur);
    (void)hipStreamWaitEvent(pc->stream, ev, 0);
    (void)hipEventDestroy(ev);
    auto g = std::make_unique<HipGraph>();
    try {
      c10::hip::HIPStreamGuard sg(c10::hip::getStreamFromExternal(pc->stream, dev));
      g->begin(pc->stream, dev);
      pc->static_out = execute(p, inputs, pc->stream);
      g->end();
    } catch (const std::exception&) {
      g->abort();
      g.release();
      p.ptr_declined = true;
      stats_.graph_failures++;
      return std::nullopt;
    }
    pc->graph = std::move(g);
    pc->cloning = cloning;
    for (auto& o : pc->static_out) {
      bool in_alias = false;
      for (auto& t : inputs) in_alias = in_alias || o.storage().is_alias_of(t.storage());
      pc->input_alias.push_back(in_alias);
      pc->base_uc.push_back(o.storage().use_count());
    }
    stats_.graphs_captured++;
    use = pc.get();
    if (!pc->cloning) register_aliases(pc.get(), alias_ptrs(pc->static_out, pc->input_alias));
    p.ptr_caps[key].push_back(std::move(pc));
    p.ptr_seen.erase(key);
  }
  use->last_use = ++p.ptr_tick;
  const int64_t t0 = now_ns();
  wait_consts(inputs[0].device(), cur);
  {
    std::lock_guard<std::mutex> cl(const_mu_);
    p.used_streams[dev].insert(cur);
  }
  use->order.before(cur);
  use->wait_uses(cur);
  use->graph->replay(cur);
  use->order.after(cur);
  std::vector<at::Tensor> outs;
  if (use->cloning) {
    outs = clone_outputs(use->static_out, cur);
    stats_.graph_busy++;
  } else {
    outs.reserve(use->static_out.size());
    for (auto& o : use->static_out) outs.push_back(o.alias());
  }
  stats_.graph_replays++;
  if (p.ptr_eager_n > 0 && p.ptr_replay_n < kGraphProbeRuns) {
    p.ptr_replay_ns += now_ns() - t0;
    if (++p.ptr_replay_n == kGraphProbeRuns && p.ptr_replay_ns * p.ptr_eager_n > p.ptr_eager_ns * p.ptr_replay_n) {
      p.ptr_declined = true;
      stats_.graphs_declined++;
    }
  }
  return outs;
}

namespace {
struct SideStreams {
  std::mutex mu;
  std::vector<hipStream_t> streams;
  std::vector<hipEvent_t> events;
  hipStream_t last_caller = nullptr;
};
SideStreams& side_streams(int dev) {
  static std::mutex m;
  static std::map<int, SideStreams*> all;
  std::lock_guard<std::mutex> lk(m);
  auto& p = all[dev];
  if (!p) p = new SideStreams();
  return *p;
}
}

std::vector<std::vector<at::Tensor>> Program::run_concurrent(
    const std::vector<std::vector<at::Tensor>>& inputs_list, int max_streams) {
  std::vector<std::vector<at::Tensor>> outs;
  if (inputs_list.empty()) return outs;
  TFA_CHECK(!inputs_list[0].empty() && inputs_list[0][0].is_cuda(), "run_concurrent: device inputs expected");
  const int dev = inputs_list[0][0].device().index();
  for (auto& ins : inputs_list)
    for (auto& t : ins)
      TFA_CHECK(t.is_cuda() && t.device().index() == dev, "run_concurrent: all inputs on one device");
  const int k = std::max(1, std::min<int>(max_streams, static_cast<int>(inputs_list.size())));
  c10::hip::HIPGuard guard(dev);
  const hipStream_t caller = c10::hip::getCurrentHIPStream(dev).stream();
  SideStreams& ss = side_streams(dev);
  std::lock_guard<std::mutex> lk(ss.mu);
  while (static_cast<int>(ss.streams.size()) < k) {
    hipStream_t st;
    TFA_CHECK(hipStreamCreateWithFlags(&st, hipStreamNonBlocking) == hipSuccess, "run_concurrent: hipStreamCreate");
    ss.streams.push_back(st);
  }
  while (ss.events.size() < ss.streams.size() + 2) {
    hipEvent_t e;
    TFA_CHECK(hipEventCreateWithFlags(&e, hipEventDisableTiming) == hipSuccess, "run_concurrent: hipEventCreate");
    ss.events.push_back(e);
  }
  TFA_CHECK(hipEventRecord(ss.events[0], caller) == hipSuccess, "run_concurrent: hipEventRecord");
  const bool other_caller = ss.last_caller && ss.last_caller != caller;
  if (other_caller)
    TFA_CHECK(hipEventRecord(ss.events[1], ss.last_caller) == hipSuccess, "run_concurrent: hipEventRecord");
  for (int i = 0; i < k; ++i) {
    TFA_CHECK(hipStreamWaitEvent(ss.streams[i], ss.events[0], 0) == hipSuccess, "run_concurrent: hipStreamWaitEvent");
    if (other_caller)
      TFA_CHECK(hipStreamWaitEvent(ss.streams[i], ss.events[1], 0) == hipSuccess, "run_concurrent: hipStreamWaitEvent");
  }
  ss.last_caller = caller;
  outs.reserve(inputs_list.size());
  for (size_t i = 0; i < inputs_list.size(); ++i) {
    const hipStream_t st = ss.streams[i % k];
    c10::hip::HIPStreamGuard sg(c10::hip::getStreamFromExternal(st, static_cast<c10::DeviceIndex>(dev)));
    outs.push_back(run(inputs_list[i]));
  }
  for (int i = 0; i < k; ++i) {
    TFA_CHECK(hipEventRecord(ss.events[2 + i], ss.streams[i]) == hipSuccess, "run_concurrent: hipEventRecord");
    TFA_CHECK(hipStreamWaitEvent(caller, ss.events[2 + i], 0) == hipSuccess, "run_concurrent: hipStreamWaitEvent");
  }
  return outs;
}

std::vector<at::Tensor> Program::run(const std::vector<at::Tensor>& inputs) {
  TFA_CHECK(host_op_error_.empty(), host_op_error_);
  auto p = plan_for(inputs);
  bool gpu = !inputs.empty() && inputs[0].is_cuda();
  void* stream = nullptr;
  std::optional<c10::hip::HIPGuard> guard;
  if (gpu) {
    guard.emplace(inputs[0].device().index());
    stream = c10::hip::getCurrentHIPStream(inputs[0].device().index()).stream();
    if (!p->stale.empty()) {
      std::lock_guard<std::mutex> lk(const_mu_);
      if (p->stale.count(inputs[0].device().index())) refresh_consts(*p, inputs[0].device().index(), stream);
    }
    if (hip_graphs_enabled()) {
      int64_t bytes = 0;
      for (auto& t : inputs) bytes += t.numel() * t.element_size();
      if (auto outs = run_ptr_graph(*p, inputs, bytes)) {
        stats_.runs++;
        return std::move(*outs);
      }
      auto& c = p->cap;
      std::lock_guard<std::mutex> lk(c.mu);
      if (p->cap_reset) {
        p->cap_reset = false;
        {
          std::lock_guard<std::mutex> pl(p->ptr_mu);
          for (auto& kv : p->ptr_caps)
            for (auto& pc : kv.second)
              if (pc->stream) (void)hipStreamSynchronize(pc->stream);
          p->ptr_caps.clear();
          p->ptr_seen.clear();
        }
        if (c.graph) {
          if (c.stream) (void)hipStreamSynchronize(c.stream);
          c.order.drain();
          c.graph.reset();
          c.static_in.clear();
          c.static_out.clear();
        }
        c.gpu_runs = 0;
        c.eager_ns = c.eager_n = c.replay_ns = c.replay_n = 0;
      }
      const bool same_dev = c.device < 0 || c.device == inputs[0].device().index();
      const bool big_enough = hip_graphs_mode() == 2 || p->steps.size() >= kGraphMinSteps;
      if (!c.failed && !c.declined && same_dev && big_enough && bytes <= hip_graph_max_bytes() && graphable(*p)) {
        if (++c.gpu_runs > kGraphWarmRuns) {
          const bool captured = c.graph != nullptr;
          const int64_t t0 = now_ns();
          auto outs = run_graph(*p, inputs);
          if (captured && c.graph && hip_graphs_mode() == 1 && c.eager_n > 0) {
            c.replay_ns += now_ns() - t0;
            if (++c.replay_n == kGraphProbeRuns && c.replay_ns * c.eager_n > c.eager_ns * c.replay_n) {
              c.declined = true;
              stats_.graphs_declined++;
            }
          }
          stats_.runs++;
          return outs;
        }
        if (c.gpu_runs > 1) {
          const int64_t t0 = now_ns();
          auto outs = execute(*p, inputs, stream);
          c.eager_ns += now_ns() - t0;
          c.eager_n++;
          stats_.runs++;
          return outs;
        }
      }
    }
  }
  auto outs = execute(*p, inputs, stream);
  stats_.runs++;
  return outs;
}

static void order_copy_after_compute(hipStream_t copy, hipStream_t compute) {
  hipEvent_t e;
  HIP_OK(hipEventCreateWithFlags(&e, hipEventDisableTiming));
  HIP_OK(hipEventRecord(e, compute));
  HIP_OK(hipStreamWaitEvent(copy, e, 0));
  HIP_OK(hipEventDestroy(e));
}

void Program::drop_pipe(bool synced) {
  if (!pipe_) return;
  if (pipe_->device >= 0) {
    c10::hip::HIPGuard guard(static_cast<c10::DeviceIndex>(pipe_->device));
    if (!synced) {
      (void)hipStreamSynchronize(copy_stream(pipe_->device, 0));
      (void)hipStreamSynchronize(copy_stream(pipe_->device, 1));
      (void)hipDeviceSynchronize();
    }
    for (hipEvent_t e : pipe_->ev_comp) (void)hipEventDestroy(e);
    for (hipEvent_t e : pipe_->ev_d2h) (void)hipEventDestroy(e);
  }
  pipe_.reset();
}

void pipeline_wait(int64_t handle) {
  if (!handle) return;
  hipEvent_t e = reinterpret_cast<hipEvent_t>(handle);
  HIP_OK(hipEventSynchronize(e));
  HIP_OK(hipEventDestroy(e));
}

int64_t Program::run_chunked(const std::vector<std::vector<at::Tensor>>& seg_inputs,
                             const std::vector<std::vector<at::Tensor>>& seg_outputs,
                             int64_t chunk_rows, int device, int depth, bool wait) {
  TFA_CHECK(host_op_error_.empty(), host_op_error_);
  TFA_CHECK(seg_inputs.size() == seg_outputs.size(), "segments mismatch");
  TFA_CHECK(chunk_rows > 0, "chunk_rows must be > 0");
  depth = std::max(2, std::min(depth, 4));
  c10::hip::HIPGuard guard(static_cast<c10::DeviceIndex>(device));
  at::Device dev(at::kCUDA, static_cast<c10::DeviceIndex>(device));
  auto compute = c10::hip::getCurrentHIPStream(device);
  auto h2d = c10::hip::getStreamFromExternal(copy_stream(device, 0), static_cast<c10::DeviceIndex>(device));
  auto d2h = c10::hip::getStreamFromExternal(copy_stream(device, 1), static_cast<c10::DeviceIndex>(device));
  auto t0 = std::chrono::steady_clock::now();

  struct Chunk {
    size_t seg;
    int64_t start, rows;
  };
  std::vector<Chunk> chunks;
  for (size_t s = 0; s < seg_inputs.size(); ++s) {
    TFA_CHECK(seg_inputs[s].size() == feed_nodes_.size(), "segment ", s, ": expected ",
              feed_nodes_.size(), " inputs");
    TFA_CHECK(seg_outputs[s].size() == fetches_.size(), "segment ", s, ": expected ",
              fetches_.size(), " outputs");
    int64_t rows = seg_inputs[s].empty() ? 0 : seg_inputs[s][0].size(0);
    for (auto& t : seg_inputs[s]) {
      TFA_CHECK(t.size(0) == rows, "segment inputs disagree on rows");
      TFA_CHECK(!t.is_cuda() && t.is_contiguous(), "run_chunked inputs must be contiguous host tensors");
    }
    for (auto& t : seg_outputs[s])
      TFA_CHECK(!t.is_cuda() && t.is_contiguous() && t.size(0) == rows,
                "run_chunked outputs must be contiguous host tensors with ", rows, " rows");
    for (int64_t st = 0; st < rows; st += chunk_rows) chunks.push_back({s, st, std::min(chunk_rows, rows - st)});
  }
  if (chunks.empty()) return 0;
  std::lock_guard<std::mutex> plk(pipe_mu_);
  size_t nin = feed_nodes_.size();
  {
    std::vector<std::vector<int64_t>> shapes;
    std::vector<at::ScalarType> dts;
    for (size_t i = 0; i < nin; ++i) {
      auto sz = seg_inputs[chunks[0].seg][i].sizes().vec();
      sz.erase(sz.begin());
      shapes.push_back(sz);
      dts.push_back(seg_inputs[chunks[0].seg][i].scalar_type());
    }
    const bool fits = pipe_ && pipe_->device == device && pipe_->depth == depth && pipe_->shapes == shapes &&
                      pipe_->dtypes == dts && pipe_->rows >= chunk_rows;
    if (!fits) {
      drop_pipe(false);
      pipe_ = std::make_unique<Pipe>();
      pipe_->device = device;
      pipe_->depth = depth;
      pipe_->rows = chunk_rows;
      pipe_->shapes = shapes;
      pipe_->dtypes = dts;
      pipe_->ring.resize(depth);
      for (int d = 0; d < depth; ++d)
        for (size_t i = 0; i < nin; ++i) {
          std::vector<int64_t> sz = shapes[i];
          sz.insert(sz.begin(), chunk_rows);
          pipe_->ring[d].push_back(dev_empty(sz, dts[i], dev, compute.stream()));
        }
      order_copy_after_compute(h2d.stream(), compute.stream());
      pipe_->ev_comp.resize(depth);
      pipe_->ev_d2h.resize(depth);
      for (int d = 0; d < depth; ++d) {
        HIP_OK(hipEventCreateWithFlags(&pipe_->ev_comp[d], hipEventDisableTiming));
        HIP_OK(hipEventCreateWithFlags(&pipe_->ev_d2h[d], hipEventDisableTiming));
      }
      pipe_->used.assign(depth, false);
    }
  }
  Pipe& P = *pipe_;
  for (size_t s = 0; s < seg_inputs.size(); ++s)
    for (size_t i = 0; i < nin; ++i) {
      auto sz = seg_inputs[s][i].sizes().vec();
      sz.erase(sz.begin());
      TFA_CHECK(sz == P.shapes[i] && seg_inputs[s][i].scalar_type() == P.dtypes[i],
                "run_chunked: segments disagree on the row shape / dtype of feed ", i);
    }
  std::vector<hipEvent_t> ev_h2d(depth);
  for (int d = 0; d < depth; ++d) HIP_OK(hipEventCreateWithFlags(&ev_h2d[d], hipEventDisableTiming));
  int64_t h2d_bytes = 0, d2h_bytes = 0;
  const bool timed = stage_timers_enabled() && wait;
  std::vector<std::array<hipEvent_t, 6>> tev;
  auto stamp = [&](size_t ci, int k, hipStream_t s) {
    if (!timed) return;
    HIP_OK(hipEventCreate(&tev[ci][k]));
    HIP_OK(hipEventRecord(tev[ci][k], s));
  };
  if (timed) tev.assign(chunks.size(), std::array<hipEvent_t, 6>{});
  const int ncomp = (pipe_compute_streams() > 1 && chunks.size() > 1) ? 2 : 1;
  hipStream_t cstr[2] = {compute.stream(), ncomp > 1 ? copy_stream(device, 2) : compute.stream()};
  hipEvent_t fork_ev = nullptr;
  if (ncomp > 1) {
    HIP_OK(hipEventCreateWithFlags(&fork_ev, hipEventDisableTiming));
    HIP_OK(hipEventRecord(fork_ev, compute.stream()));
    HIP_OK(hipStreamWaitEvent(cstr[1], fork_ev, 0));
  }
  for (size_t ci = 0; ci < chunks.size(); ++ci) {
    const hipStream_t cs = cstr[ci % ncomp];
    const Chunk& ch = chunks[ci];
    const int slot = static_cast<int>(P.next++ % depth);
    if (P.used[slot]) {
      HIP_OK(hipStreamWaitEvent(h2d.stream(), P.ev_comp[slot], 0));
      HIP_OK(hipStreamWaitEvent(h2d.stream(), P.ev_d2h[slot], 0));
    }
    std::vector<at::Tensor> dev_in;
    stamp(ci, 0, h2d.stream());
    for (size_t i = 0; i < nin; ++i) {
      const at::Tensor& src = seg_inputs[ch.seg][i];
      int64_t row_bytes = src.numel() / std::max<int64_t>(src.size(0), 1) * src.element_size();
      at::Tensor dst = P.ring[slot][i].narrow(0, 0, ch.rows);
      const char* sp = static_cast<const char*>(src.data_ptr()) + ch.start * row_bytes;
      if (ch.rows * row_bytes)
        HIP_OK(hipMemcpyAsync(dst.data_ptr(), sp, ch.rows * row_bytes, hipMemcpyHostToDevice, h2d.stream()));
      h2d_bytes += ch.rows * row_bytes;
      dev_in.push_back(dst);
    }
    stamp(ci, 1, h2d.stream());
    HIP_OK(hipEventRecord(ev_h2d[slot], h2d.stream()));
    HIP_OK(hipStreamWaitEvent(cs, ev_h2d[slot], 0));
    std::vector<at::Tensor> outs;
    stamp(ci, 2, cs);
    {
      RangeGuard rg("chunk_compute");
      auto p = plan_for(dev_in);
      outs = execute(*p, dev_in, cs);
    }
    stamp(ci, 3, cs);
    HIP_OK(hipEventRecord(P.ev_comp[slot], cs));
    HIP_OK(hipStreamWaitEvent(d2h.stream(), P.ev_comp[slot], 0));
    stamp(ci, 4, d2h.stream());
    for (size_t j = 0; j < outs.size(); ++j) {
      at::Tensor o = outs[j];
      const at::Tensor& dst = seg_outputs[ch.seg][j];
      int64_t row_bytes = dst.numel() / std::max<int64_t>(dst.size(0), 1) * dst.element_size();
      TFA_CHECK(o.size(0) == ch.rows && o.numel() * o.element_size() == ch.rows * row_bytes,
                "fetch '", fetch_names_[j], "' produced ", o.size(0), " rows for a chunk of ", ch.rows);
      if (!o.is_cuda()) o = o.to(dev);
      char* dp = static_cast<char*>(dst.data_ptr()) + ch.start * row_bytes;
      if (ch.rows * row_bytes)
        HIP_OK(hipMemcpyAsync(dp, o.data_ptr(), ch.rows * row_bytes, hipMemcpyDeviceToHost, d2h.stream()));
      dev_record_stream(o, d2h.stream());
      d2h_bytes += ch.rows * row_bytes;
    }
    stamp(ci, 5, d2h.stream());
    HIP_OK(hipEventRecord(P.ev_d2h[slot], d2h.stream()));
    P.used[slot] = true;
    stats_.chunks++;
  }
  if (ncomp > 1) {
    HIP_OK(hipEventRecord(fork_ev, cstr[1]));
    HIP_OK(hipStreamWaitEvent(compute.stream(), fork_ev, 0));
    HIP_OK(hipEventDestroy(fork_ev));
  }
  int64_t handle = 0;
  if (wait) {
    HIP_OK(hipStreamSynchronize(h2d.stream()));
    HIP_OK(hipStreamSynchronize(compute.stream()));
    HIP_OK(hipStreamSynchronize(d2h.stream()));
    drop_pipe(true);
  } else {
    hipEvent_t done;
    HIP_OK(hipEventCreateWithFlags(&done, hipEventDisableTiming));
    HIP_OK(hipEventRecord(done, d2h.stream()));
    handle = reinterpret_cast<int64_t>(done);
  }
  for (int d = 0; d < depth; ++d) hipEventDestroy(ev_h2d[d]);
  double stage_ms[3] = {0, 0, 0};
  for (auto& e : tev) {
    for (int k = 0; k < 3; ++k) {
      float ms = 0.f;
      if (hipEventElapsedTime(&ms, e[2 * k], e[2 * k + 1]) == hipSuccess) stage_ms[k] += ms;
    }
    for (hipEvent_t ev : e) hipEventDestroy(ev);
  }
  auto t1 = std::chrono::steady_clock::now();
  stats_.runs++;
  stats_.h2d_bytes += h2d_bytes;
  stats_.d2h_bytes += d2h_bytes;
  stats_.wall_ms += std::chrono::duration<double, std::milli>(t1 - t0).count();
  stats_.h2d_ms += stage_ms[0];
  stats_.compute_ms += stage_ms[1];
  stats_.d2h_ms += stage_ms[2];
  return handle;
}

std::vector<at::Tensor> Program::run_chunked_reduce(const std::vector<std::vector<at::Tensor>>& seg_inputs,
                                                    int64_t chunk_rows, int device, int depth) {
  TFA_CHECK(host_op_error_.empty(), host_op_error_);
  TFA_CHECK(chunk_rows > 0, "chunk_rows must be > 0");
  depth = std::max(2, std::min(depth, 4));
  c10::hip::HIPGuard guard(static_cast<c10::DeviceIndex>(device));
  at::Device dev(at::kCUDA, static_cast<c10::DeviceIndex>(device));
  auto compute = c10::hip::getCurrentHIPStream(device);
  auto h2d = c10::hip::getStreamFromExternal(copy_stream(device, 0), static_cast<c10::DeviceIndex>(device));
  auto t0 = std::chrono::steady_clock::now();
  struct Chunk {
    size_t seg;
    int64_t start, rows;
  };
  std::vector<Chunk> chunks;
  for (size_t s = 0; s < seg_inputs.size(); ++s) {
    TFA_CHECK(seg_inputs[s].size() == feed_nodes_.size(), "segment ", s, ": expected ", feed_nodes_.size(), " inputs");
    const int64_t rows = seg_inputs[s].empty() ? 0 : seg_inputs[s][0].size(0);
    for (auto& t : seg_inputs[s]) {
      TFA_CHECK(t.size(0) == rows, "segment inputs disagree on rows");
      TFA_CHECK(!t.is_cuda() && t.is_contiguous(), "run_chunked_reduce inputs must be contiguous host tensors");
    }
    for (int64_t st = 0; st < rows; st += chunk_rows) chunks.push_back({s, st, std::min(chunk_rows, rows - st)});
  }
  TFA_CHECK(!chunks.empty(), "run_chunked_reduce: no rows");
  const size_t nin = feed_nodes_.size();
  std::vector<std::vector<at::Tensor>> ring(depth);
  for (int d = 0; d < depth; ++d)
    for (size_t i = 0; i < nin; ++i) {
      auto sz = seg_inputs[0][i].sizes().vec();
      sz[0] = chunk_rows;
      ring[d].push_back(dev_empty(sz, seg_inputs[0][i].scalar_type(), dev, compute.stream()));
    }
  order_copy_after_compute(h2d.stream(), compute.stream());
  std::vector<hipEvent_t> ev_h2d(depth), ev_comp(depth);
  for (int d = 0; d < depth; ++d) {
    HIP_OK(hipEventCreateWithFlags(&ev_h2d[d], hipEventDisableTiming));
    HIP_OK(hipEventCreateWithFlags(&ev_comp[d], hipEventDisableTiming));
  }
  std::vector<bool> used(depth, false);
  std::vector<at::Tensor> acc;
  int64_t h2d_bytes = 0;
  for (size_t ci = 0; ci < chunks.size(); ++ci) {
    const Chunk& ch = chunks[ci];
    const int slot = static_cast<int>(ci % depth);
    if (used[slot]) HIP_OK(hipStreamWaitEvent(h2d.stream(), ev_comp[slot], 0));
    std::vector<at::Tensor> dev_in;
    for (size_t i = 0; i < nin; ++i) {
      const at::Tensor& src = seg_inputs[ch.seg][i];
      const int64_t row_bytes = src.numel() / std::max<int64_t>(src.size(0), 1) * src.element_size();
      at::Tensor dst = ring[slot][i].narrow(0, 0, ch.rows);
      const char* sp = static_cast<const char*>(src.data_ptr()) + ch.start * row_bytes;
      if (ch.rows * row_bytes)
        HIP_OK(hipMemcpyAsync(dst.data_ptr(), sp, ch.rows * row_bytes, hipMemcpyHostToDevice, h2d.stream()));
      h2d_bytes += ch.rows * row_bytes;
      dev_in.push_back(dst);
    }
    HIP_OK(hipEventRecord(ev_h2d[slot], h2d.stream()));
    HIP_OK(hipStreamWaitEvent(compute.stream(), ev_h2d[slot], 0));
    std::vector<at::Tensor> outs;
    {
      RangeGuard rg("chunk_reduce");
      auto p = plan_for(dev_in);
      outs = execute(*p, dev_in, compute.stream());
    }
    if (acc.empty()) {
      for (auto& o : outs) {
        auto sz = o.sizes().vec();
        sz.insert(sz.begin(), static_cast<int64_t>(chunks.size()));
        acc.push_back(dev_empty(sz, o.scalar_type(), dev, compute.stream()));
      }
    }
    for (size_t j = 0; j < outs.size(); ++j) {
      at::Tensor o = outs[j].is_cuda() ? outs[j].contiguous() : outs[j].to(dev);
      at::Tensor dst = acc[j].select(0, static_cast<int64_t>(ci));
      TFA_CHECK(o.numel() == dst.numel(), "fetch '", fetch_names_[j], "' changed shape between chunks");
      const int64_t nb = o.numel() * o.element_size();
      if (nb) HIP_OK(hipMemcpyAsync(dst.data_ptr(), o.data_ptr(), nb, hipMemcpyDeviceToDevice, compute.stream()));
    }
    HIP_OK(hipEventRecord(ev_comp[slot], compute.stream()));
    used[slot] = true;
    stats_.chunks++;
  }
  HIP_OK(hipStreamSynchronize(h2d.stream()));
  for (int d = 0; d < depth; ++d) {
    hipEventDestroy(ev_h2d[d]);
    hipEventDestroy(ev_comp[d]);
  }
  auto t1 = std::chrono::steady_clock::now();
  stats_.runs++;
  stats_.h2d_bytes += h2d_bytes;
  stats_.wall_ms += std::chrono::duration<double, std::milli>(t1 - t0).count();
  return acc;
}

std::vector<std::string> Program::fused_sources(const std::vector<at::Tensor>& inputs) {
  auto p = build_plan(inputs, true);
  std::vector<std::string> out;
  for (auto& f : p->fused_regions) out.push_back(f->region.source);
  return out;
}

ExecStats Program::stats() const { return stats_; }
void Program::reset_stats() { stats_ = ExecStats(); }

std::string Program::describe_plan(const std::vector<at::Tensor>& inputs, bool as_gpu) {
  auto p = as_gpu ? build_plan(inputs, true) : plan_for(inputs);
  std::ostringstream os;
  os << "plan: " << p->steps.size() << " steps, " << p->const_slots.size() << " constants, "
     << p->fused << " fused epilogues, " << p->fused_regions.size() << " fused regions";
  if (p->fused_siblings) os << ", " << p->fused_siblings << " sibling convs fused";
  if (p->wino_convs) os << ", " << p->wino_convs << " Winograd filters";
  {
    const std::string why = graph_blocker(*p);
    os << (why.empty() ? ", graphable" : ", not graphable (" + why + ")");
  }
  os << "\n";
  for (auto& st : p->steps) {
    const Node& nd = g_->node(st.node);
    if (st.kind == Step::FUSED) {
      const FusedRegion& rg = p->fused_regions[st.fused]->region;
      os << "  FUSED" << (rg.kind == 1 ? "-ROWRED " : " ") << nd.name << " [" << rg.expr << "] "
         << rg.leaves.size() << " inputs " << rg.outputs.size() << " outputs " << st.out_info[0].shape.str();
      os << (rg.idx64 ? " idx64" : " idx32");
      if (rg.kind == 1) os << (rg.wave ? " wave" : " thread");
      os << " leaves[";
      static const char* leaf_kinds[] = {"contiguous", "scalar", "strided"};
      for (size_t k = 0; k < rg.leaves.size(); ++k) os << (k ? "," : "") << leaf_kinds[rg.leaves[k].kind];
      os << "]\n";
      continue;
    }
    os << "  " << (st.kind == Step::GEMM ? "GEMM" : st.kind == Step::CONV ? "CONV" : "OP  ") << ' '
       << nd.op << ' ' << nd.name;
    if (st.out_node != st.node) os << " -> " << g_->node(st.out_node).name;
    if (st.bias_slot >= 0) os << " +bias";
    if (st.act) os << " +" << act_name(st.act);
    if (!st.epi.empty()) {
      static const char* codes[] = {"add", "sub", "rsub", "mul", "div", "rdiv", "max", "min", "act", "neg", "square", "abs"};
      static const char* kinds[] = {"", "scalar", "scalar", "col", "row", "full"};
      os << " +epi[";
      for (size_t k = 0; k < st.epi.size(); ++k) {
        const auto& e = st.epi[k];
        os << (k ? "," : "") << (e.code == k::EPI_ACT ? act_name(e.act) : codes[e.code]);
        if (e.kind != k::EPO_NONE) os << ":" << kinds[e.kind];
      }
      os << "]";
    }
    if (st.alias_slot >= 0) os << " ->concat-slice@" << st.alias_offset;
    if (st.wino_slot >= 0) os << " +winograd";
    if (st.pool2) os << " +maxpool2x2";
    if (st.pool_in[0]) os << " +maxpool" << st.pool_in[0] << "x" << st.pool_in[1] << "/" << st.pool_in[2] << "-in";
    if (!st.sibs.empty()) {
      os << " siblings[";
      for (size_t k = 0; k < st.sibs.size(); ++k) {
        const auto& sb = st.sibs[k];
        os << (k ? "," : "") << g_->node(sb.node).name << ":" << sb.oc;
        if (sb.act) os << "+" << act_name(sb.act);
        if (sb.alias_slot >= 0) os << "->concat-slice@" << sb.alias_offset;
      }
      os << "]";
    }
    if (!st.preplaced.empty()) {
      int n = 0;
      for (char c : st.preplaced) n += c;
      os << " (" << n << " inputs written in place)";
    }
    os << ' ' << st.out_info[0].shape.str() << '\n';
  }
  return os.str();
}

namespace {
class PinnedPool {
 public:
  static PinnedPool& get() {
    static PinnedPool* p = new PinnedPool();
    return *p;
  }
  void* alloc(size_t bytes, size_t* rounded) {
    size_t r = (bytes + kGran - 1) / kGran * kGran;
    *rounded = r;
    {
      std::lock_guard<std::mutex> lk(mu_);
      auto it = free_.find(r);
      if (it != free_.end()) {
        void* p = it->second;
        free_.erase(it);
        cached_ -= r;
        return p;
      }
    }
    if (live_.load() + cached_ + r > limit_) trim(limit_ > live_.load() + r ? limit_ - live_.load() - r : 0);
    void* p = nullptr;
    hipError_t e = hipHostMalloc(&p, r, hipHostMallocDefault);
    if (e != hipSuccess) {
      trim(0);
      HIP_OK(hipHostMalloc(&p, r, hipHostMallocDefault));
    }
    return p;
  }
  void note_live(size_t r, bool add) {
    const size_t now = add ? (live_ += r) : (live_ -= r);
    size_t pk = peak_.load();
    while (now > pk && !peak_.compare_exchange_weak(pk, now)) {
    }
  }
  void release(void* p, size_t r) {
    std::lock_guard<std::mutex> lk(mu_);
    free_.emplace(r, p);
    cached_ += r;
    while (cached_ > limit_ && !free_.empty()) {
      auto it = std::prev(free_.end());
      cached_ -= it->first;
      hipHostFree(it->second);
      free_.erase(it);
    }
  }
  void trim(size_t keep) {
    std::lock_guard<std::mutex> lk(mu_);
    while (cached_ > keep && !free_.empty()) {
      auto it = free_.begin();
      cached_ -= it->first;
      hipHostFree(it->second);
      free_.erase(it);
    }
  }
  size_t cached() const { return cached_; }
  size_t live() const { return live_.load(); }
  size_t peak() const { return peak_.load(); }
  size_t limit() const { return limit_; }

 private:
  PinnedPool() { limit_ = default_limit(); }
  static size_t default_limit() {
    if (const char* e = std::getenv("TFA_PINNED_POOL_MB"))
      if (std::atoll(e) > 0) return static_cast<size_t>(std::atoll(e)) << 20;
    const long pages = sysconf(_SC_PHYS_PAGES), psz = sysconf(_SC_PAGE_SIZE);
    size_t ram = pages > 0 && psz > 0 ? static_cast<size_t>(pages) * static_cast<size_t>(psz) : (size_t(64) << 30);
    int local = 1;
    if (const char* lw = std::getenv("LOCAL_WORLD_SIZE")) local = std::max(1, std::atoi(lw));
    return std::min(size_t(64) << 30, ram / static_cast<size_t>(local) / 2);
  }
  static constexpr size_t kGran = size_t(2) << 20;
  std::mutex mu_;
  std::multimap<size_t, void*> free_;
  size_t cached_ = 0;
  std::atomic<size_t> live_{0}, peak_{0};
  size_t limit_;
};
}

at::Tensor empty_pinned(const std::vector<int64_t>& sizes, at::ScalarType dt) {
  int64_t n = 1;
  for (auto s : sizes) n *= s;
  size_t bytes = static_cast<size_t>(std::max<int64_t>(n, 1)) * c10::elementSize(dt);
  size_t r = 0;
  void* p = PinnedPool::get().alloc(bytes, &r);
  PinnedPool::get().note_live(r, true);
  return at::from_blob(p, sizes,
                       [r](void* q) {
                         PinnedPool::get().note_live(r, false);
                         PinnedPool::get().release(q, r);
                       },
                       at::TensorOptions().dtype(dt));
}

void trim_pinned_pool() { PinnedPool::get().trim(0); }
size_t pinned_pool_cached_bytes() { return PinnedPool::get().cached(); }
std::vector<size_t> pinned_pool_stats() {
  auto& p = PinnedPool::get();
  return {p.limit(), p.cached(), p.live(), p.peak()};
}

void pin_host_tensor(const at::Tensor& t) {
  TFA_CHECK(!t.is_cuda(), "pin_host_tensor needs a host tensor");
  size_t bytes = t.numel() * t.element_size();
  if (!bytes) return;
  HIP_OK(hipHostRegister(t.data_ptr(), bytes, hipHostRegisterDefault));
}

void unpin_host_tensor(const at::Tensor& t) {
  if (t.numel()) hipHostUnregister(t.data_ptr());
}

}
```

csrc/runtime/executor.h:

```cpp
#pragma once

#include <ATen/ATen.h>
#include <hip/hip_runtime.h>

#include <map>
#include <tuple>
#include <memory>
#include <mutex>
#include <optional>
#include <string>
#include <vector>

#include "../ir/graph.h"

namespace tfa {

struct MonoidInfo {
  std::string fetch;
  std::string placeholder;
  std::string op;
};

struct ExecStats {
  int64_t runs = 0;
  int64_t kernels = 0;
  int64_t plans_built = 0;
  int64_t plans_adopted = 0;
  int64_t h2d_bytes = 0;
  int64_t d2h_bytes = 0;
  int64_t chunks = 0;
  double h2d_ms = 0, compute_ms = 0, d2h_ms = 0, wall_ms = 0;
  double plan_ms = 0;
  double exec_ms = 0;
  int64_t graphs_captured = 0, graph_replays = 0, graph_failures = 0, graphs_declined = 0;
  int64_t graph_busy = 0;
};

class Program {
 public:
  Program(std::shared_ptr<Graph> g, const std::vector<std::string>& fetches,
          const std::vector<std::string>& feeds);
  ~Program();

  const std::vector<std::string>& fetch_names() const { return fetch_names_; }
  const std::vector<std::string>& feed_names() const { return feed_names_; }

  Graph::Infos analyze(const std::map<std::string, TensorInfo>& feed_infos) const;
  bool row_separable(const std::map<std::string, TensorInfo>& feed_infos) const;
  std::vector<MonoidInfo> monoids() const;

  bool adopt(Program& old);
  std::shared_ptr<Program> rebind(const std::map<std::string, at::Tensor>& values);

  std::vector<at::Tensor> run(const std::vector<at::Tensor>& inputs);

  std::vector<std::vector<at::Tensor>> run_concurrent(const std::vector<std::vector<at::Tensor>>& inputs_list,
                                                      int max_streams = 4);

  int64_t run_chunked(const std::vector<std::vector<at::Tensor>>& seg_inputs,
                      const std::vector<std::vector<at::Tensor>>& seg_outputs, int64_t chunk_rows,
                      int device, int depth, bool wait = true);

  void release_pipeline() {
    std::lock_guard<std::mutex> lk(pipe_mu_);
    drop_pipe(false);
  }

  std::vector<at::Tensor> run_chunked_reduce(const std::vector<std::vector<at::Tensor>>& seg_inputs,
                                             int64_t chunk_rows, int device, int depth);

  ExecStats stats() const;
  void reset_stats();
  std::string describe_plan(const std::vector<at::Tensor>& inputs, bool as_gpu = false);
  std::vector<std::string> fused_sources(const std::vector<at::Tensor>& inputs);

 private:
  std::string host_op_error_;
  struct Step;
  struct Plan;
 public:
  struct AliasUseSink {
    virtual ~AliasUseSink() = default;
    virtual void record_use(hipStream_t s) = 0;
  };

 private:
  std::shared_ptr<Plan> plan_for(const std::vector<at::Tensor>& inputs);
  std::shared_ptr<Plan> build_plan(const std::vector<at::Tensor>& inputs, bool force_gpu);
  std::vector<at::Tensor> execute(Plan& p, const std::vector<at::Tensor>& inputs, void* stream);
  at::Tensor device_const(Plan& p, int slot, const at::Device& dev, void* stream);
  void upload_consts(Plan& p, std::map<int, at::Tensor>& m, const at::Device& dev, void* stream);
  void wait_consts(const at::Device& dev, void* stream);
  void refresh_consts(Plan& p, int di, void* stream);
  bool graphable(const Plan& p) const;
  std::string graph_blocker(const Plan& p) const;
  std::vector<at::Tensor> run_graph(Plan& p, const std::vector<at::Tensor>& inputs);
  std::optional<std::vector<at::Tensor>> run_ptr_graph(Plan& p, const std::vector<at::Tensor>& inputs,
                                                       int64_t bytes);

  std::shared_ptr<Graph> g_;
  std::vector<std::string> fetch_names_, feed_names_;
  std::vector<TensorRef> fetches_;
  std::vector<int> feed_nodes_;
  std::vector<int> order_;
  std::mutex mu_;
  static constexpr size_t kMaxPlans = 256;
  std::map<std::string, std::shared_ptr<Plan>> plans_;
  std::mutex const_mu_;
  std::map<std::tuple<int, int, int>, at::Tensor> graph_consts_;
  std::map<std::pair<int, void*>, void*> const_events_;
  ExecStats stats_;
  struct Pipe {
    int device = -1, depth = 0;
    int64_t rows = 0;
    std::vector<std::vector<int64_t>> shapes;
    std::vector<at::ScalarType> dtypes;
    std::vector<std::vector<at::Tensor>> ring;
    std::vector<hipEvent_t> ev_comp, ev_d2h;
    std::vector<bool> used;
    int64_t next = 0;
  };
  std::mutex pipe_mu_;
  std::unique_ptr<Pipe> pipe_;
  void drop_pipe(bool synced);
};

struct StepTiming {
  std::string node, op, label;
  double flops, bytes;
  float ms;
};
void set_step_timing(bool on);
bool step_timing();
std::vector<StepTiming> read_step_timing();

void pipeline_wait(int64_t handle);

at::Tensor empty_pinned(const std::vector<int64_t>& sizes, at::ScalarType dt);
void trim_pinned_pool();
size_t pinned_pool_cached_bytes();
std::vector<size_t> pinned_pool_stats();
void pin_host_tensor(const at::Tensor& t);
void unpin_host_tensor(const at::Tensor& t);
hipStream_t copy_stream(int device, int which);
void set_debug_sync(bool on);
bool get_debug_sync();

}
```

tensorframes_amd/config.py:

```python
from __future__ import annotations

import dataclasses
import os


def _env(name, default, cast):
    v = os.environ.get(name)
    if v is None:
        return default
    if cast is bool:
        return v.lower() in ("1", "true", "yes", "on")
    return cast(v)


@dataclasses.dataclass
class Config:
    device: str = dataclasses.field(default_factory=lambda: _env("TFA_DEVICE", "auto", str))
    collect_to: str = dataclasses.field(default_factory=lambda: _env("TFA_COLLECT_TO", "all", str))
    graph_rewrites: bool = dataclasses.field(default_factory=lambda: _env("TFA_GRAPH_REWRITES", True, bool))
    plan_reuse: bool = dataclasses.field(default_factory=lambda: _env("TFA_PLAN_REUSE", True, bool))
    chunk_bytes: int = dataclasses.field(default_factory=lambda: _env("TFA_CHUNK_BYTES", 128 << 20, int))
    min_pipeline_chunks: int = dataclasses.field(default_factory=lambda: _env("TFA_MIN_PIPELINE_CHUNKS", 16, int))
    pipeline_depth: int = dataclasses.field(default_factory=lambda: _env("TFA_PIPELINE_DEPTH", 3, int))
    min_chunked_rows: int = dataclasses.field(default_factory=lambda: _env("TFA_MIN_CHUNKED_ROWS", 65536, int))
    min_chunked_bytes: int = dataclasses.field(default_factory=lambda: _env("TFA_MIN_CHUNKED_BYTES", 32 << 20, int))
    stream_group_bytes: int = dataclasses.field(default_factory=lambda: _env("TFA_STREAM_GROUP_BYTES", 4 << 30, int))
    pinned_outputs: bool = dataclasses.field(default_factory=lambda: _env("TFA_PINNED_OUTPUTS", True, bool))
    pinned_min_bytes: int = dataclasses.field(default_factory=lambda: _env("TFA_PINNED_MIN_BYTES", 1 << 20, int))
    map_rows_gpu_min_elems: int = dataclasses.field(default_factory=lambda: _env("TFA_MAP_ROWS_GPU_MIN", 16384, int))
    map_rows_vectorize: bool = dataclasses.field(default_factory=lambda: _env("TFA_MAP_ROWS_VECTORIZE", True, bool))
    map_rows_batch_rows: int = dataclasses.field(default_factory=lambda: _env("TFA_MAP_ROWS_BATCH", 256, int))
    map_rows_batched_prestage: bool = dataclasses.field(
        default_factory=lambda: _env("TFA_MAP_ROWS_BATCHED_PRESTAGE", True, bool))
    native_jpeg_decode: bool = dataclasses.field(default_factory=lambda: _env("TFA_NATIVE_JPEG", True, bool))
    string_key_hash: bool = dataclasses.field(default_factory=lambda: _env("TFA_STRING_KEY_HASH", True, bool))
    decode_threads: int = dataclasses.field(default_factory=lambda: _env("TFA_DECODE_THREADS", 0, int))
    task_retries: int = dataclasses.field(default_factory=lambda: _env("TFA_TASK_RETRIES", 0, int))
    collective_timeout_s: float = dataclasses.field(default_factory=lambda: _env("TFA_COLLECTIVE_TIMEOUT_S", 600.0, float))
    collective_timeout_exit: bool = dataclasses.field(default_factory=lambda: _env("TFA_COLLECTIVE_TIMEOUT_EXIT", True, bool))
    shm_collectives: bool = dataclasses.field(default_factory=lambda: _env("TFA_SHM_COLLECTIVES", True, bool))
    shm_slot_bytes: int = dataclasses.field(default_factory=lambda: _env("TFA_SHM_SLOT_BYTES", 8 << 20, int))
    cpu_parallel_min_elems: int = dataclasses.field(default_factory=lambda: _env("TFA_CPU_PARALLEL_MIN_ELEMS", 4_000_000, int))
    precision: str = dataclasses.field(default_factory=lambda: _env("TFA_PRECISION", "f32", str))
    force_collectives: bool = dataclasses.field(default_factory=lambda: _env("TFA_FORCE_COLLECTIVES", False, bool))
    collective_backend: str = dataclasses.field(default_factory=lambda: _env("TFA_COLLECTIVE_BACKEND", "engine", str))
    oneshot_allreduce: bool = dataclasses.field(default_factory=lambda: _env("TFA_ONESHOT_ALLREDUCE", True, bool))
    eager_device_map: bool = dataclasses.field(default_factory=lambda: _env("TFA_EAGER_DEVICE_MAP", True, bool))
    eager_device_map_bytes: int = dataclasses.field(
        default_factory=lambda: _env("TFA_EAGER_DEVICE_MAP_BYTES", 1 << 30, int))
    concurrent_partitions: bool = dataclasses.field(default_factory=lambda: _env("TFA_CONCURRENT_PARTITIONS", False, bool))
    concurrent_large_partitions: bool = dataclasses.field(
        default_factory=lambda: _env("TFA_CONCURRENT_LARGE", True, bool))
    concurrent_large_bytes: int = dataclasses.field(
        default_factory=lambda: _env("TFA_CONCURRENT_LARGE_BYTES", 64 << 20, int))
    concurrent_large_streams: int = dataclasses.field(
        default_factory=lambda: _env("TFA_CONCURRENT_LARGE_STREAMS", 2, int))
    wino_5x5: bool = dataclasses.field(default_factory=lambda: _env("TFA_WINO_5X5", False, bool))
    pool_conv_fusion: bool = dataclasses.field(default_factory=lambda: _env("TFA_POOL_CONV_FUSION", True, bool))
    debug_sync: bool = dataclasses.field(default_factory=lambda: _env("TFA_DEBUG_SYNC", False, bool))


config = Config()


def set_config(**kw):
    if "precision" in kw and kw["precision"] not in PRECISION_MODES:
        raise ValueError(f"precision must be one of {sorted(PRECISION_MODES)}, got {kw['precision']!r}")
    for k, v in kw.items():
        if not hasattr(config, k):
            raise AttributeError(f"unknown config key {k}")
        setattr(config, k, v)
    if "debug_sync" in kw:
        os.environ["TFA_DEBUG_SYNC"] = "1" if kw["debug_sync"] else "0"
        from ._native import _C
        _C.set_debug_sync(bool(kw["debug_sync"]))
    if "precision" in kw:
        apply_precision()
    if "pool_conv_fusion" in kw:
        from ._native import _C
        from . import engine
        _C.set_pool_conv_fusion(bool(kw["pool_conv_fusion"]))
        engine.clear_program_cache()
    if "wino_5x5" in kw:
        from ._native import _C
        from . import engine
        _C.set_wino_5x5(bool(kw["wino_5x5"]))
        engine.clear_program_cache()


PRECISION_MODES = {"f32": 0, "bf16": 1, "bf16x3": 2}


def apply_precision():
    if config.precision not in PRECISION_MODES:
        raise ValueError(f"precision must be one of {sorted(PRECISION_MODES)}, got {config.precision!r}")
    from ._native import _C
    from . import engine
    _C.set_f32_precision(PRECISION_MODES[config.precision])
    engine.clear_program_cache()
```

Before: 23.47 million rows/s.

## Pack sparse chunk outputs on device before D2H and expand on host threads

Adds a GPU kernel that compacts each output chunk into a bitmask of nonzero 32-bit words plus the nonzero values, with per-tile offsets taken from an atomic cursor. A lander thread waits on the copy event and hands the packed buffer to a host worker pool, which expands it with scalar, AVX2 or AVX-512 code. Outputs whose packed size exceeds a set fraction of the dense size fall back to plain copies. The aim is to shrink device-to-host traffic for ReLU outputs, which hold many zeros. The cost is an extra device kernel, host CPU expansion work and more synchronisation in the chunk pipeline.

```diff
diff --git a/csrc/bindings.cpp b/csrc/bindings.cpp
--- a/csrc/bindings.cpp
+++ b/csrc/bindings.cpp
@@ -12,6 +12,7 @@
 #include "runtime/fusion.h"
 #include "runtime/jit.h"
 #include "runtime/jpeg_decode.h"
+#include "runtime/unpack.h"
 #include <rocprofiler-sdk-roctx/roctx.h>
 
 namespace py = pybind11;
@@ -302,7 +303,9 @@
         d["plans_adopted"] = s.plans_adopted;
         d["h2d_bytes"] = s.h2d_bytes;
         d["d2h_bytes"] = s.d2h_bytes;
+        d["d2h_dense_bytes"] = s.d2h_dense_bytes;
         d["chunks"] = s.chunks;
+        d["chunks_packed"] = s.chunks_packed;
         d["wall_ms"] = s.wall_ms;
         d["plan_ms"] = s.plan_ms;
         d["exec_ms"] = s.exec_ms;
@@ -2115,6 +2118,71 @@
   }, py::arg("columns"), "row concatenations of several columns into one pool buffer (views of it)");
   m.def("pipeline_wait", &pipeline_wait, py::arg("handle"), py::call_guard<py::gil_scoped_release>(),
         "wait for a run_chunked(wait=False) completion handle (and release it)");
+  m.def("set_pack_outputs", &set_pack_outputs, py::arg("on"),
+        "run_chunked packs eligible fetches before their D2H copy (config.pack_outputs)");
+  m.def("pack_outputs", &pack_outputs);
+  m.def("set_pack_dense_fraction", &set_pack_dense_fraction, py::arg("t"),
+        "packed / dense size ratio above which a fetch goes back to plain copies (<= 0: the built-in value)");
+  m.def("pack_dense_fraction", &pack_dense_fraction);
+  m.def("pack_layout", [](int64_t rows, int64_t wpr) {
+    const PackLayout L = pack_layout(rows, wpr);
+    py::dict d;
+    d["tile_rows"] = kPackTileRows;
+    d["tiles"] = L.tiles;
+    d["mask_words"] = L.mask_words;
+    d["mask_off"] = L.mask_off;
+    d["values_off"] = L.values_off;
+    d["max_bytes"] = L.max_bytes;
+    return d;
+  }, py::arg("rows"), py::arg("wpr"), "byte layout of a packed rows x wpr buffer (kernels/pack_layout.h)");
+  m.def("pack_words", [](const at::Tensor& src, int64_t rows, int64_t wpr) {
+    TFA_CHECK(src.is_cuda() && src.is_contiguous(), "pack_words: contiguous device tensor expected");
+    TFA_CHECK(rows >= 0 && wpr >= 0 && static_cast<int64_t>(src.numel() * src.element_size()) == rows * wpr * 4,
+              "pack_words: the tensor is not ", rows, " x ", wpr, " words");
+    c10::hip::HIPGuard guard(src.device().index());
+    at::Tensor out = pool_empty({static_cast<int64_t>(k::pack_words_max_bytes(rows, wpr))},
+                                at::TensorOptions().dtype(at::kByte).device(src.device()));
+    k::pack_words(src.data_ptr(), rows, wpr, out.data_ptr(), c10::hip::getCurrentHIPStream(src.device().index()).stream());
+    return out;
+  }, py::arg("src"), py::arg("rows"), py::arg("wpr"),
+        "the packed form (uint8 [max_bytes]; the first 8 bytes are the value word count) of a device buffer");
+  m.def("unpack_words", [](const at::Tensor& packed, at::Tensor& out, int64_t rows, int64_t wpr, int threads) {
+    TFA_CHECK(!packed.is_cuda() && !out.is_cuda() && packed.is_contiguous() && out.is_contiguous(),
+              "unpack_words: contiguous host tensors expected");
+    const PackLayout L = pack_layout(rows, wpr);
+    const size_t have = packed.numel() * packed.element_size();
+    TFA_CHECK(have >= L.values_off, "unpack_words: packed buffer shorter than its header and mask");
+    const uint64_t total = rows && wpr ? *static_cast<const uint64_t*>(packed.data_ptr()) : 0;
+    TFA_CHECK(total <= static_cast<uint64_t>(rows * wpr) && have >= L.values_off + total * 4,
+              "unpack_words: packed buffer shorter than its ", total, " values");
+    TFA_CHECK(static_cast<int64_t>(out.numel() * out.element_size()) == rows * wpr * 4,
+              "unpack_words: the output is not ", rows, " x ", wpr, " words");
+    py::gil_scoped_release nogil;
+    if (threads <= 0) {
+      unpack::unpack_buffer(packed.data_ptr(), out.data_ptr(), rows, wpr, 0, L.tiles);
+    } else {
+      unpack::Pool pool(threads);
+      pool.post_unpack(packed.data_ptr(), out.data_ptr(), rows, wpr)->wait();
+    }
+  }, py::arg("packed"), py::arg("out"), py::arg("rows"), py::arg("wpr"), py::arg("threads") = 0,
+        "expand a packed host buffer into `out` (threads > 0: on a pool of that many workers)");
+  m.def("unpack_force_variant", &unpack::force_variant, py::arg("variant"),
+        "test hook: -1 auto, 0 scalar, 1 AVX2, 2 AVX-512");
+  m.def("unpack_variant_available", &unpack::variant_available, py::arg("variant"));
+  m.def("unpack_current_variant", &unpack::current_variant);
+  m.def("unpack_default_threads", &unpack::default_threads);
+  m.def("unpack_pool_raise", [](int threads, int parts, int bad_part) {
+    py::gil_scoped_release nogil;
+    unpack::Pool pool(threads);
+    pool.post(parts, [bad_part](int p) {
+      if (p == bad_part) throw std::runtime_error("unpack pool test: part " + std::to_string(p) + " failed");
+    })->wait();
+  }, py::arg("threads"), py::arg("parts"), py::arg("bad_part"),
+        "test hook: a pool job whose part `bad_part` throws; the waiter (this call) re-raises it");
+  py::module_::import("atexit").attr("register")(py::cpp_function([] {
+    py::gil_scoped_release nogil;
+    shutdown_pack_runtime();
+  }));
   m.def("device_empty", [](const std::vector<int64_t>& sizes, at::ScalarType dt, int device) {
     c10::hip::HIPGuard guard(static_cast<c10::DeviceIndex>(device));
     return pool_empty(sizes, at::TensorOptions().dtype(dt).device(at::kCUDA, static_cast<c10::DeviceIndex>(device)));
diff --git a/csrc/kernels/kernels.h b/csrc/kernels/kernels.h
--- a/csrc/kernels/kernels.h
+++ b/csrc/kernels/kernels.h
@@ -138,6 +138,9 @@
 void compact_gather(const PackCols& src, const PackCols& dst, const uint8_t* mask, int64_t n, int64_t total,
                     const void* workspace, int64_t* index, hipStream_t s);
 
+size_t pack_words_max_bytes(int64_t rows, int64_t wpr);
+void pack_words(const void* src, int64_t rows, int64_t wpr, void* packed, hipStream_t s);
+
 constexpr int kMaxSortKeys = 8;
 struct SortKeys {
   int n = 0;
diff --git a/csrc/kernels/pack_layout.h b/csrc/kernels/pack_layout.h
--- /dev/null
+++ b/csrc/kernels/pack_layout.h
@@ -0,0 +1,33 @@
+#pragma once
+
+#include <cstddef>
+#include <cstdint>
+
+namespace tfa {
+
+constexpr int kPackTileRows = 32;
+
+struct PackLayout {
+  int64_t rows = 0, wpr = 0;
+  int64_t tiles = 0;
+  int64_t mask_words = 0;
+  size_t mask_off = 0;
+  size_t values_off = 0;
+  size_t max_bytes = 0;
+};
+
+inline PackLayout pack_layout(int64_t rows, int64_t wpr) {
+  PackLayout L;
+  L.rows = rows;
+  L.wpr = wpr;
+  L.tiles = (rows + kPackTileRows - 1) / kPackTileRows;
+  L.mask_words = (rows * wpr + 31) / 32;
+  const size_t hdr = (static_cast<size_t>(1 + 2 * L.tiles) * 8 + 63) / 64 * 64;
+  const size_t msk = (static_cast<size_t>(L.mask_words) * 4 + 63) / 64 * 64;
+  L.mask_off = hdr;
+  L.values_off = hdr + msk;
+  L.max_bytes = L.values_off + static_cast<size_t>(rows) * static_cast<size_t>(wpr) * 4;
+  return L;
+}
+
+}
diff --git a/csrc/kernels/pack_words.hip b/csrc/kernels/pack_words.hip
--- /dev/null
+++ b/csrc/kernels/pack_words.hip
@@ -0,0 +1,115 @@
+#include "hip_common.h"
+#include "pack_layout.h"
+
+namespace tfa {
+namespace k {
+
+namespace {
+
+constexpr int kPT = 256;
+constexpr int kPW = kPT / kWave;
+constexpr int kPU = 4;
+
+__global__ __launch_bounds__(kPT) void pack_words_kernel(const uint32_t* __restrict__ src, int64_t rows, int64_t wpr,
+                                                         uint64_t* __restrict__ header, uint32_t* __restrict__ mask,
+                                                         uint32_t* __restrict__ values) {
+  __shared__ uint32_t wtot[kPW];
+  __shared__ unsigned long long sbase;
+  const int tid = threadIdx.x, lane = tid & (kWave - 1), wave = tid / kWave;
+  const int64_t t = blockIdx.x;
+  const int64_t r0 = t * kPackTileRows;
+  const int64_t r1 = r0 + kPackTileRows < rows ? r0 + kPackTileRows : rows;
+  const int64_t e0 = r0 * wpr;
+  const uint32_t n = (uint32_t)((r1 - r0) * wpr);
+  const uint32_t ngroups = (n + 63u) / 64u, per = (ngroups + kPW - 1) / kPW;
+  const uint32_t g0 = min((uint32_t)wave * per, ngroups), g1 = min(g0 + per, ngroups);
+  const uint32_t* __restrict__ s = src + e0;
+  uint32_t* __restrict__ mw = mask + e0 / 32;
+  const unsigned long long below = (1ull << lane) - 1ull;
+
+  auto put_mask = [&](uint32_t g, unsigned long long b) {
+    if (lane < 2 && g * 64u + (uint32_t)lane * 32u < n) mw[2 * g + lane] = (uint32_t)(b >> (32 * lane));
+  };
+
+  uint32_t cnt = 0;
+  uint32_t g = g0;
+  for (; g + kPU <= g1 && (g + kPU) * 64u <= n; g += kPU) {
+    uint32_t w[kPU];
+#pragma unroll
+    for (int j = 0; j < kPU; ++j) w[j] = s[(g + j) * 64u + lane];
+#pragma unroll
+    for (int j = 0; j < kPU; ++j) {
+      const unsigned long long b = __ballot(w[j] != 0u);
+      put_mask(g + j, b);
+      cnt += __popcll(b);
+    }
+  }
+  for (; g < g1; ++g) {
+    const uint32_t i = g * 64u + lane;
+    const uint32_t w = i < n ? s[i] : 0u;
+    const unsigned long long b = __ballot(w != 0u);
+    put_mask(g, b);
+    cnt += __popcll(b);
+  }
+  if (lane == 0) wtot[wave] = cnt;
+  __syncthreads();
+  if (tid == 0) {
+    unsigned long long total = 0;
+#pragma unroll
+    for (int w = 0; w < kPW; ++w) total += wtot[w];
+    const unsigned long long base = atomicAdd(reinterpret_cast<unsigned long long*>(header), total);
+    header[1 + 2 * t] = base;
+    header[2 + 2 * t] = total;
+    sbase = base;
+  }
+  __syncthreads();
+  unsigned long long pos = sbase;
+#pragma unroll
+  for (int w = 0; w < kPW; ++w)
+    if (w < wave) pos += wtot[w];
+  uint32_t* __restrict__ vout = values + pos;
+
+  uint32_t run = 0;
+  g = g0;
+  for (; g + kPU <= g1 && (g + kPU) * 64u <= n; g += kPU) {
+    uint32_t w[kPU];
+#pragma unroll
+    for (int j = 0; j < kPU; ++j) w[j] = s[(g + j) * 64u + lane];
+#pragma unroll
+    for (int j = 0; j < kPU; ++j) {
+      const unsigned long long b = __ballot(w[j] != 0u);
+      if (w[j] != 0u) vout[run + __popcll(b & below)] = w[j];
+      run += __popcll(b);
+    }
+  }
+  for (; g < g1; ++g) {
+    const uint32_t i = g * 64u + lane;
+    const uint32_t w = i < n ? s[i] : 0u;
+    const unsigned long long b = __ballot(w != 0u);
+    if (w != 0u) vout[run + __popcll(b & below)] = w;
+    run += __popcll(b);
+  }
+}
+
+}
+
+size_t pack_words_max_bytes(int64_t rows, int64_t wpr) { return pack_layout(rows, wpr).max_bytes; }
+
+void pack_words(const void* src, int64_t rows, int64_t wpr, void* packed, hipStream_t s) {
+  TFA_CHECK(rows >= 0 && wpr >= 0, "pack_words: negative shape");
+  TFA_CHECK((reinterpret_cast<uintptr_t>(src) & 3) == 0 && (reinterpret_cast<uintptr_t>(packed) & 63) == 0,
+            "pack_words: source must be 4-byte, destination 64-byte aligned");
+  TFA_CHECK(hipMemsetAsync(packed, 0, 8, s) == hipSuccess, "pack_words: memset of the cursor failed");
+  if (rows == 0 || wpr == 0) return;
+  const PackLayout L = pack_layout(rows, wpr);
+  TFA_CHECK(L.tiles < (int64_t(1) << 31), "pack_words: more than 2^31 tiles");
+  TFA_CHECK(wpr * kPackTileRows < (int64_t(1) << 31), "pack_words: rows of ", wpr, " words are too wide");
+  char* p = static_cast<char*>(packed);
+  hipLaunchKernelGGL(pack_words_kernel, dim3((unsigned)L.tiles), dim3(kPT), 0, s, static_cast<const uint32_t*>(src),
+                     rows, wpr, reinterpret_cast<uint64_t*>(p), reinterpret_cast<uint32_t*>(p + L.mask_off),
+                     reinterpret_cast<uint32_t*>(p + L.values_off));
+  TFA_LAUNCH_CHECK("pack_words_kernel");
+}
+
+}
+}
diff --git a/csrc/runtime/executor.cpp b/csrc/runtime/executor.cpp
--- a/csrc/runtime/executor.cpp
+++ b/csrc/runtime/executor.cpp
@@ -14,6 +14,9 @@
 #include <array>
 #include <atomic>
 #include <chrono>
+#include <condition_variable>
+#include <deque>
+#include <thread>
 #include <unistd.h>
 #include <cstdlib>
 #include <set>
@@ -24,6 +27,7 @@
 #include "fusion.h"
 #include "hip_graph.h"
 #include "jit.h"
+#include "unpack.h"
 
 namespace tfa {
 
@@ -2125,6 +2129,151 @@
   HIP_OK(hipEventDestroy(e));
 }
 
+
+constexpr double kPackDenseFraction = 0.782;
+std::atomic<double> g_pack_dense_fraction{kPackDenseFraction};
+constexpr int kPackStages = 3;
+
+struct PackLanding {
+  struct Task {
+    const void* packed;
+    void* out;
+    int64_t rows, wpr;
+  };
+  hipEvent_t ev = nullptr;
+  std::vector<Task> tasks;
+
+  void wait() {
+    std::unique_lock<std::mutex> lk(mu);
+    cv.wait(lk, [&] { return posted; });
+    for (auto& j : jobs) {
+      if (!j) continue;
+      try {
+        j->wait();
+      } catch (const std::exception& e) {
+        if (error.empty()) error = e.what();
+      }
+      j.reset();
+    }
+    TFA_CHECK(error.empty(), "packed output expansion failed: ", error);
+  }
+
+  std::mutex mu;
+  std::condition_variable cv;
+  bool posted = false;
+  std::string error;
+  std::vector<std::shared_ptr<unpack::Job>> jobs;
+};
+
+namespace {
+
+class PackLander {
+ public:
+  static PackLander& get() {
+    std::lock_guard<std::mutex> lk(inst_mu());
+    if (!inst()) inst().reset(new PackLander());
+    return *inst();
+  }
+  static void shutdown() {
+    std::unique_ptr<PackLander> p;
+    {
+      std::lock_guard<std::mutex> lk(inst_mu());
+      p = std::move(inst());
+    }
+    p.reset();
+  }
+  void submit(std::shared_ptr<PackLanding> l) {
+    {
+      std::lock_guard<std::mutex> lk(mu_);
+      q_.push_back(std::move(l));
+    }
+    cv_.notify_one();
+  }
+  ~PackLander() {
+    {
+      std::lock_guard<std::mutex> lk(mu_);
+      stop_ = true;
+    }
+    cv_.notify_all();
+    thread_.join();
+  }
+
+ private:
+  PackLander() : thread_([this] { loop(); }) {}
+  static std::mutex& inst_mu() {
+    static std::mutex m;
+    return m;
+  }
+  static std::unique_ptr<PackLander>& inst() {
+    static std::unique_ptr<PackLander> p;
+    return p;
+  }
+  void loop() {
+    for (;;) {
+      std::shared_ptr<PackLanding> l;
+      {
+        std::unique_lock<std::mutex> lk(mu_);
+        cv_.wait(lk, [&] { return stop_ || !q_.empty(); });
+        if (q_.empty()) return;
+        l = std::move(q_.front());
+        q_.pop_front();
+      }
+      std::string err;
+      std::vector<std::shared_ptr<unpack::Job>> jobs;
+      const hipError_t e = hipEventSynchronize(l->ev);
+      if (e != hipSuccess) {
+        err = std::string("D2H of a packed chunk: ") + hipGetErrorString(e);
+      } else {
+        try {
+          for (auto& t : l->tasks) jobs.push_back(unpack::global_pool().post_unpack(t.packed, t.out, t.rows, t.wpr));
+        } catch (const std::exception& ex) {
+          err = ex.what();
+        }
+      }
+      {
+        std::lock_guard<std::mutex> lk(l->mu);
+        l->jobs = std::move(jobs);
+        l->error = err;
+        l->posted = true;
+      }
+      l->cv.notify_all();
+    }
+  }
+  std::mutex mu_;
+  std::condition_variable cv_;
+  std::deque<std::shared_ptr<PackLanding>> q_;
+  bool stop_ = false;
+  std::thread thread_;
+};
+
+std::atomic<int>& pack_outputs_state() {
+  static std::atomic<int> v([] {
+    const char* e = std::getenv("TFA_PACK_OUTPUTS");
+    if (!e) return 1;
+    std::string s(e);
+    for (auto& c : s) c = static_cast<char>(std::tolower(static_cast<unsigned char>(c)));
+    return (s == "1" || s == "true" || s == "yes" || s == "on") ? 1 : 0;
+  }());
+  return v;
+}
+
+struct PipeHandle {
+  hipEvent_t done = nullptr;
+  std::vector<std::shared_ptr<PackLanding>> landings;
+};
+
+}
+
+void set_pack_outputs(bool on) { pack_outputs_state().store(on ? 1 : 0); }
+void set_pack_dense_fraction(double t) { g_pack_dense_fraction.store(t > 0 ? t : kPackDenseFraction); }
+double pack_dense_fraction() { return g_pack_dense_fraction.load(); }
+bool pack_outputs() { return pack_outputs_state().load() != 0; }
+
+void shutdown_pack_runtime() {
+  PackLander::shutdown();
+  unpack::shutdown_pool();
+}
+
 void Program::drop_pipe(bool synced) {
   if (!pipe_) return;
   if (pipe_->device >= 0) {
@@ -2134,17 +2283,35 @@
       (void)hipStreamSynchronize(copy_stream(pipe_->device, 1));
       (void)hipDeviceSynchronize();
     }
+    for (auto& l : pipe_->landing)
+      if (l) {
+        try {
+          l->wait();
+        } catch (const std::exception&) {
+        }
+      }
     for (hipEvent_t e : pipe_->ev_comp) (void)hipEventDestroy(e);
     for (hipEvent_t e : pipe_->ev_d2h) (void)hipEventDestroy(e);
+    for (hipEvent_t e : pipe_->ev_land) (void)hipEventDestroy(e);
   }
   pipe_.reset();
 }
 
 void pipeline_wait(int64_t handle) {
   if (!handle) return;
-  hipEvent_t e = reinterpret_cast<hipEvent_t>(handle);
-  HIP_OK(hipEventSynchronize(e));
-  HIP_OK(hipEventDestroy(e));
+  std::unique_ptr<PipeHandle> h(reinterpret_cast<PipeHandle*>(handle));
+  const hipError_t e = hipEventSynchronize(h->done);
+  (void)hipEventDestroy(h->done);
+  std::string err;
+  for (auto& l : h->landings) {
+    try {
+      l->wait();
+    } catch (const std::exception& ex) {
+      if (err.empty()) err = ex.what();
+    }
+  }
+  HIP_OK(e);
+  TFA_CHECK(err.empty(), err);
 }
 
 int64_t Program::run_chunked(const std::vector<std::vector<at::Tensor>>& seg_inputs,
@@ -2218,6 +2385,7 @@
         HIP_OK(hipEventCreateWithFlags(&pipe_->ev_d2h[d], hipEventDisableTiming));
       }
       pipe_->used.assign(depth, false);
+      pipe_->d2h_issued.assign(depth, true);
     }
   }
   Pipe& P = *pipe_;
@@ -2230,7 +2398,41 @@
     }
   std::vector<hipEvent_t> ev_h2d(depth);
   for (int d = 0; d < depth; ++d) HIP_OK(hipEventCreateWithFlags(&ev_h2d[d], hipEventDisableTiming));
-  int64_t h2d_bytes = 0, d2h_bytes = 0;
+  int64_t h2d_bytes = 0, d2h_bytes = 0, d2h_dense_bytes = 0;
+  const size_t nf = fetches_.size();
+  if (pack_dense_.size() != nf) pack_dense_.assign(nf, 0);
+  std::vector<char> packing(nf, 0), probe_only(nf, 0);
+  std::vector<int64_t> fetch_wpr(nf, 0);
+  if (pack_outputs()) {
+    bool any = false;
+    for (size_t j = 0; j < nf; ++j) {
+      const at::Tensor& dst = seg_outputs[chunks[0].seg][j];
+      const int64_t rb = dst.numel() / std::max<int64_t>(dst.size(0), 1) * dst.element_size();
+      if (rb <= 0 || rb % 4 != 0) continue;
+      fetch_wpr[j] = rb / 4;
+      packing[j] = 1;
+      probe_only[j] = pack_dense_[j];
+      any = true;
+    }
+    if (any && P.packed.empty()) {
+      P.packed.assign(depth, std::vector<at::Tensor>(nf));
+      P.stage.assign(kPackStages, std::vector<at::Tensor>(nf));
+      P.landing.assign(kPackStages, nullptr);
+      P.ev_land.resize(kPackStages);
+      for (auto& e : P.ev_land) HIP_OK(hipEventCreateWithFlags(&e, hipEventDisableTiming));
+      P.counts = empty_pinned({static_cast<int64_t>(depth * nf)}, at::kLong);
+    }
+    for (size_t j = 0; j < nf; ++j) {
+      if (!packing[j]) continue;
+      const int64_t need = static_cast<int64_t>(pack_layout(P.rows, fetch_wpr[j]).max_bytes);
+      if (!P.packed[0][j].defined()) {
+        for (int d = 0; d < depth; ++d) P.packed[d][j] = dev_empty({need}, at::kByte, dev, compute.stream());
+        for (int k = 0; k < kPackStages; ++k) P.stage[k][j] = empty_pinned({need}, at::kByte);
+      } else if (P.packed[0][j].numel() < need) {
+        packing[j] = 0;
+      }
+    }
+  }
   const bool timed = stage_timers_enabled() && wait;
   std::vector<std::array<hipEvent_t, 6>> tev;
   auto stamp = [&](size_t ci, int k, hipStream_t s) {
@@ -2247,14 +2449,91 @@
     HIP_OK(hipEventRecord(fork_ev, compute.stream()));
     HIP_OK(hipStreamWaitEvent(cstr[1], fork_ev, 0));
   }
+  struct PendingD2H {
+    bool active = false;
+    size_t ci = 0;
+    int slot = 0;
+    std::vector<at::Tensor> outs;
+    std::vector<char> packed;
+    bool any_packed = false;
+  };
+  std::vector<std::shared_ptr<PackLanding>> call_landings;
+  uint64_t* const counts = P.counts.defined() ? reinterpret_cast<uint64_t*>(P.counts.data_ptr()) : nullptr;
+  auto issue_d2h = [&](PendingD2H& pd) {
+    const Chunk& ch = chunks[pd.ci];
+    const int slot = pd.slot;
+    std::shared_ptr<PackLanding> landing;
+    int stage = -1;
+    if (pd.any_packed) {
+      HIP_OK(hipEventSynchronize(P.ev_comp[slot]));
+      stage = static_cast<int>(P.stage_next++ % kPackStages);
+      if (P.landing[stage]) {
+        std::shared_ptr<PackLanding> prev = std::move(P.landing[stage]);
+        prev->wait();
+      }
+      landing = std::make_shared<PackLanding>();
+      landing->ev = P.ev_land[stage];
+    }
+    HIP_OK(hipStreamWaitEvent(d2h.stream(), P.ev_comp[slot], 0));
+    stamp(pd.ci, 4, d2h.stream());
+    for (size_t j = 0; j < pd.outs.size(); ++j) {
+      at::Tensor o = pd.outs[j];
+      const at::Tensor& dst = seg_outputs[ch.seg][j];
+      int64_t row_bytes = dst.numel() / std::max<int64_t>(dst.size(0), 1) * dst.element_size();
+      char* dp = static_cast<char*>(dst.data_ptr()) + ch.start * row_bytes;
+      d2h_dense_bytes += ch.rows * row_bytes;
+      if (pd.packed[j]) {
+        const PackLayout L = pack_layout(ch.rows, fetch_wpr[j]);
+        const uint64_t total = counts[slot * nf + j];
+        TFA_CHECK(total <= static_cast<uint64_t>(ch.rows * fetch_wpr[j]), "fetch '", fetch_names_[j],
+                  "': packed ", total, " words of ", ch.rows * fetch_wpr[j]);
+        const size_t bytes = L.values_off + static_cast<size_t>(total) * 4;
+        HIP_OK(hipMemcpyAsync(P.stage[stage][j].data_ptr(), P.packed[slot][j].data_ptr(), bytes,
+                              hipMemcpyDeviceToHost, d2h.stream()));
+        d2h_bytes += static_cast<int64_t>(bytes);
+        landing->tasks.push_back({P.stage[stage][j].data_ptr(), dp, ch.rows, fetch_wpr[j]});
+        const bool dense =
+            static_cast<double>(bytes) > g_pack_dense_fraction.load() * static_cast<double>(ch.rows * row_bytes);
+        if (dense) {
+          packing[j] = 0;
+          pack_dense_[j] = 1;
+        } else if (pack_dense_[j]) {
+          pack_dense_[j] = 0;
+          probe_only[j] = 0;
+          packing[j] = 1;
+        }
+        continue;
+      }
+      if (!o.is_cuda()) o = o.to(dev);
+      if (ch.rows * row_bytes)
+        HIP_OK(hipMemcpyAsync(dp, o.data_ptr(), ch.rows * row_bytes, hipMemcpyDeviceToHost, d2h.stream()));
+      dev_record_stream(o, d2h.stream());
+      d2h_bytes += ch.rows * row_bytes;
+    }
+    stamp(pd.ci, 5, d2h.stream());
+    HIP_OK(hipEventRecord(P.ev_d2h[slot], d2h.stream()));
+    P.d2h_issued[slot] = true;
+    if (landing) {
+      HIP_OK(hipEventRecord(landing->ev, d2h.stream()));
+      P.landing[stage] = landing;
+      call_landings.push_back(landing);
+      PackLander::get().submit(landing);
+      stats_.chunks_packed++;
+    }
+    pd.outs.clear();
+    pd.active = false;
+  };
+  PendingD2H lagged;
   for (size_t ci = 0; ci < chunks.size(); ++ci) {
     const hipStream_t cs = cstr[ci % ncomp];
     const Chunk& ch = chunks[ci];
     const int slot = static_cast<int>(P.next++ % depth);
     if (P.used[slot]) {
+      TFA_CHECK(P.d2h_issued[slot], "run_chunked: slot ", slot, " reused before its D2H was issued");
       HIP_OK(hipStreamWaitEvent(h2d.stream(), P.ev_comp[slot], 0));
       HIP_OK(hipStreamWaitEvent(h2d.stream(), P.ev_d2h[slot], 0));
     }
+    P.d2h_issued[slot] = false;
     std::vector<at::Tensor> dev_in;
     stamp(ci, 0, h2d.stream());
     for (size_t i = 0; i < nin; ++i) {
@@ -2278,27 +2557,44 @@
       outs = execute(*p, dev_in, cs);
     }
     stamp(ci, 3, cs);
-    HIP_OK(hipEventRecord(P.ev_comp[slot], cs));
-    HIP_OK(hipStreamWaitEvent(d2h.stream(), P.ev_comp[slot], 0));
-    stamp(ci, 4, d2h.stream());
+    PendingD2H pd;
+    pd.active = true;
+    pd.ci = ci;
+    pd.slot = slot;
+    pd.packed.assign(nf, 0);
     for (size_t j = 0; j < outs.size(); ++j) {
-      at::Tensor o = outs[j];
+      const at::Tensor& o = outs[j];
       const at::Tensor& dst = seg_outputs[ch.seg][j];
       int64_t row_bytes = dst.numel() / std::max<int64_t>(dst.size(0), 1) * dst.element_size();
       TFA_CHECK(o.size(0) == ch.rows && o.numel() * o.element_size() == ch.rows * row_bytes,
                 "fetch '", fetch_names_[j], "' produced ", o.size(0), " rows for a chunk of ", ch.rows);
-      if (!o.is_cuda()) o = o.to(dev);
-      char* dp = static_cast<char*>(dst.data_ptr()) + ch.start * row_bytes;
-      if (ch.rows * row_bytes)
-        HIP_OK(hipMemcpyAsync(dp, o.data_ptr(), ch.rows * row_bytes, hipMemcpyDeviceToHost, d2h.stream()));
-      dev_record_stream(o, d2h.stream());
-      d2h_bytes += ch.rows * row_bytes;
-    }
-    stamp(ci, 5, d2h.stream());
-    HIP_OK(hipEventRecord(P.ev_d2h[slot], d2h.stream()));
+      if (!packing[j] || ch.rows == 0 || row_bytes != 4 * fetch_wpr[j]) continue;
+      bool plain = o.is_cuda() && o.is_contiguous();
+      for (size_t i = 0; plain && i < nin; ++i) {
+        const char* r0 = static_cast<const char*>(P.ring[slot][i].data_ptr());
+        const char* op = static_cast<const char*>(o.data_ptr());
+        if (op >= r0 && op < r0 + P.ring[slot][i].numel() * P.ring[slot][i].element_size()) plain = false;
+      }
+      if (!plain) continue;
+      if (!pd.any_packed && P.used[slot])
+        HIP_OK(hipStreamWaitEvent(cs, P.ev_d2h[slot], 0));
+      k::pack_words(o.data_ptr(), ch.rows, fetch_wpr[j], P.packed[slot][j].data_ptr(), cs);
+      HIP_OK(hipMemcpyAsync(counts + slot * nf + j, P.packed[slot][j].data_ptr(), 8, hipMemcpyDeviceToHost, cs));
+      pd.packed[j] = 1;
+      pd.any_packed = true;
+      if (probe_only[j]) packing[j] = 0;
+    }
+    pd.outs = std::move(outs);
+    HIP_OK(hipEventRecord(P.ev_comp[slot], cs));
     P.used[slot] = true;
     stats_.chunks++;
-  }
+    if (lagged.active) issue_d2h(lagged);
+    if (pd.any_packed)
+      lagged = std::move(pd);
+    else
+      issue_d2h(pd);
+  }
+  if (lagged.active) issue_d2h(lagged);
   if (ncomp > 1) {
     HIP_OK(hipEventRecord(fork_ev, cstr[1]));
     HIP_OK(hipStreamWaitEvent(compute.stream(), fork_ev, 0));
@@ -2309,12 +2605,22 @@
     HIP_OK(hipStreamSynchronize(h2d.stream()));
     HIP_OK(hipStreamSynchronize(compute.stream()));
     HIP_OK(hipStreamSynchronize(d2h.stream()));
+    std::string err;
+    for (auto& l : call_landings) {
+      try {
+        l->wait();
+      } catch (const std::exception& ex) {
+        if (err.empty()) err = ex.what();
+      }
+    }
     drop_pipe(true);
+    TFA_CHECK(err.empty(), err);
   } else {
-    hipEvent_t done;
-    HIP_OK(hipEventCreateWithFlags(&done, hipEventDisableTiming));
-    HIP_OK(hipEventRecord(done, d2h.stream()));
-    handle = reinterpret_cast<int64_t>(done);
+    auto h = std::make_unique<PipeHandle>();
+    HIP_OK(hipEventCreateWithFlags(&h->done, hipEventDisableTiming));
+    HIP_OK(hipEventRecord(h->done, d2h.stream()));
+    h->landings = std::move(call_landings);
+    handle = reinterpret_cast<int64_t>(h.release());
   }
   for (int d = 0; d < depth; ++d) hipEventDestroy(ev_h2d[d]);
   double stage_ms[3] = {0, 0, 0};
@@ -2329,6 +2635,7 @@
   stats_.runs++;
   stats_.h2d_bytes += h2d_bytes;
   stats_.d2h_bytes += d2h_bytes;
+  stats_.d2h_dense_bytes += d2h_dense_bytes;
   stats_.wall_ms += std::chrono::duration<double, std::milli>(t1 - t0).count();
   stats_.h2d_ms += stage_ms[0];
   stats_.compute_ms += stage_ms[1];
diff --git a/csrc/runtime/executor.h b/csrc/runtime/executor.h
--- a/csrc/runtime/executor.h
+++ b/csrc/runtime/executor.h
@@ -28,13 +28,17 @@
   int64_t plans_adopted = 0;
   int64_t h2d_bytes = 0;
   int64_t d2h_bytes = 0;
+  int64_t d2h_dense_bytes = 0;
   int64_t chunks = 0;
+  int64_t chunks_packed = 0;
   double h2d_ms = 0, compute_ms = 0, d2h_ms = 0, wall_ms = 0;
   double plan_ms = 0;
   double exec_ms = 0;
   int64_t graphs_captured = 0, graph_replays = 0, graph_failures = 0, graphs_declined = 0;
   int64_t graph_busy = 0;
 };
+
+struct PackLanding;
 
 class Program {
  public:
@@ -119,9 +123,17 @@
     std::vector<hipEvent_t> ev_comp, ev_d2h;
     std::vector<bool> used;
     int64_t next = 0;
+    std::vector<bool> d2h_issued;
+    std::vector<std::vector<at::Tensor>> packed;
+    at::Tensor counts;
+    std::vector<std::vector<at::Tensor>> stage;
+    std::vector<hipEvent_t> ev_land;
+    std::vector<std::shared_ptr<PackLanding>> landing;
+    int64_t stage_next = 0;
   };
   std::mutex pipe_mu_;
   std::unique_ptr<Pipe> pipe_;
+  std::vector<char> pack_dense_;
   void drop_pipe(bool synced);
 };
 
@@ -135,6 +147,11 @@
 std::vector<StepTiming> read_step_timing();
 
 void pipeline_wait(int64_t handle);
+void set_pack_outputs(bool on);
+bool pack_outputs();
+void set_pack_dense_fraction(double t);
+double pack_dense_fraction();
+void shutdown_pack_runtime();
 
 at::Tensor empty_pinned(const std::vector<int64_t>& sizes, at::ScalarType dt);
 void trim_pinned_pool();
diff --git a/csrc/runtime/unpack.cpp b/csrc/runtime/unpack.cpp
--- /dev/null
+++ b/csrc/runtime/unpack.cpp
@@ -0,0 +1,307 @@
+#include "unpack.h"
+
+#include <algorithm>
+#include <atomic>
+#include <cstdlib>
+#include <cstring>
+#include <stdexcept>
+#include <string>
+
+#if defined(__linux__)
+#include <sched.h>
+#endif
+#if defined(__x86_64__)
+#include <immintrin.h>
+#define TFA_UNPACK_X86 1
+#else
+#define TFA_UNPACK_X86 0
+#endif
+
+namespace tfa {
+namespace unpack {
+
+namespace {
+
+using TileFn = void (*)(const uint32_t* mask, const uint32_t* v, const uint32_t* vend, uint32_t* out, int64_t n);
+
+inline uint32_t tail_bits(int64_t n) { return n >= 32 ? 0xffffffffu : ((1u << n) - 1u); }
+
+void scalar_from(const uint32_t* mask, const uint32_t* v, uint32_t* out, int64_t n, int64_t j0) {
+  for (int64_t j = j0; j * 32 < n; ++j) {
+    const int64_t left = n - j * 32;
+    const int w = static_cast<int>(std::min<int64_t>(32, left));
+    uint32_t m = mask[j] & tail_bits(left);
+    uint32_t* o = out + j * 32;
+    std::memset(o, 0, static_cast<size_t>(w) * 4);
+    while (m) {
+      o[__builtin_ctz(m)] = *v++;
+      m &= m - 1;
+    }
+  }
+}
+
+void tile_scalar(const uint32_t* mask, const uint32_t* v, const uint32_t*, uint32_t* out, int64_t n) {
+  scalar_from(mask, v, out, n, 0);
+}
+
+#if TFA_UNPACK_X86
+__attribute__((target("avx512f,popcnt"))) void tile_avx512(const uint32_t* mask, const uint32_t* v,
+                                                           const uint32_t*, uint32_t* out, int64_t n) {
+  const int64_t full = n / 32;
+  const bool stream = (reinterpret_cast<uintptr_t>(out) & 63) == 0;
+  if (stream) {
+    for (int64_t j = 0; j < full; ++j) {
+      const uint32_t m = mask[j];
+      const __mmask16 lo = static_cast<__mmask16>(m & 0xffffu), hi = static_cast<__mmask16>(m >> 16);
+      const __m512i a = _mm512_maskz_expandloadu_epi32(lo, v);
+      v += __builtin_popcount(m & 0xffffu);
+      const __m512i b = _mm512_maskz_expandloadu_epi32(hi, v);
+      v += __builtin_popcount(m >> 16);
+      _mm512_stream_si512(reinterpret_cast<__m512i*>(out + j * 32), a);
+      _mm512_stream_si512(reinterpret_cast<__m512i*>(out + j * 32 + 16), b);
+    }
+    _mm_sfence();
+  } else {
+    for (int64_t j = 0; j < full; ++j) {
+      const uint32_t m = mask[j];
+      const __mmask16 lo = static_cast<__mmask16>(m & 0xffffu), hi = static_cast<__mmask16>(m >> 16);
+      const __m512i a = _mm512_maskz_expandloadu_epi32(lo, v);
+      v += __builtin_popcount(m & 0xffffu);
+      const __m512i b = _mm512_maskz_expandloadu_epi32(hi, v);
+      v += __builtin_popcount(m >> 16);
+      _mm512_storeu_si512(out + j * 32, a);
+      _mm512_storeu_si512(out + j * 32 + 16, b);
+    }
+  }
+  scalar_from(mask, v, out, n, full);
+}
+
+struct Avx2Lut {
+  alignas(32) uint32_t idx[256][8];
+  Avx2Lut() {
+    for (int m = 0; m < 256; ++m) {
+      int k = 0;
+      for (int i = 0; i < 8; ++i) idx[m][i] = ((m >> i) & 1) ? static_cast<uint32_t>(k++) : 0u;
+    }
+  }
+};
+
+__attribute__((target("avx2,popcnt"))) void tile_avx2(const uint32_t* mask, const uint32_t* v, const uint32_t* vend,
+                                                      uint32_t* out, int64_t n) {
+  static const Avx2Lut lut;
+  const int64_t full = n / 32;
+  const bool stream = (reinterpret_cast<uintptr_t>(out) & 31) == 0;
+  const __m256i bit = _mm256_setr_epi32(1, 2, 4, 8, 16, 32, 64, 128);
+  for (int64_t j = 0; j < full; ++j) {
+    const uint32_t m = mask[j];
+    for (int q = 0; q < 4; ++q) {
+      const uint32_t mb = (m >> (8 * q)) & 0xffu;
+      uint32_t* o = out + j * 32 + q * 8;
+      const int pc = __builtin_popcount(mb);
+      if (v + 8 <= vend) {
+        const __m256i src = _mm256_loadu_si256(reinterpret_cast<const __m256i*>(v));
+        const __m256i perm =
+            _mm256_permutevar8x32_epi32(src, _mm256_load_si256(reinterpret_cast<const __m256i*>(lut.idx[mb])));
+        const __m256i keep = _mm256_cmpeq_epi32(_mm256_and_si256(_mm256_set1_epi32(static_cast<int>(mb)), bit), bit);
+        const __m256i r = _mm256_and_si256(perm, keep);
+        if (stream)
+          _mm256_stream_si256(reinterpret_cast<__m256i*>(o), r);
+        else
+          _mm256_storeu_si256(reinterpret_cast<__m256i*>(o), r);
+      } else {
+        const uint32_t* vv = v;
+        for (int i = 0; i < 8; ++i) o[i] = ((mb >> i) & 1u) ? *vv++ : 0u;
+      }
+      v += pc;
+    }
+  }
+  if (stream) _mm_sfence();
+  scalar_from(mask, v, out, n, full);
+}
+#endif
+
+std::atomic<int> g_forced{kAuto};
+
+int best_variant() {
+#if TFA_UNPACK_X86
+  static const int best = [] {
+    if (__builtin_cpu_supports("avx512f") && __builtin_cpu_supports("popcnt")) return static_cast<int>(kAvx512);
+    if (__builtin_cpu_supports("avx2") && __builtin_cpu_supports("popcnt")) return static_cast<int>(kAvx2);
+    return static_cast<int>(kScalar);
+  }();
+  return best;
+#else
+  return kScalar;
+#endif
+}
+
+TileFn tile_fn(int v) {
+#if TFA_UNPACK_X86
+  if (v == kAvx512) return tile_avx512;
+  if (v == kAvx2) return tile_avx2;
+#endif
+  (void)v;
+  return tile_scalar;
+}
+
+}
+
+bool variant_available(int v) {
+  if (v == kScalar || v == kAuto) return true;
+#if TFA_UNPACK_X86
+  if (v == kAvx2) return __builtin_cpu_supports("avx2") && __builtin_cpu_supports("popcnt");
+  if (v == kAvx512) return __builtin_cpu_supports("avx512f") && __builtin_cpu_supports("popcnt");
+#endif
+  return false;
+}
+
+void force_variant(int v) {
+  if (v < kAuto || v > kAvx512 || !variant_available(v))
+    throw std::runtime_error("unpack: variant " + std::to_string(v) + " is not available on this CPU");
+  g_forced.store(v);
+}
+
+int current_variant() {
+  const int f = g_forced.load();
+  return f == kAuto ? best_variant() : f;
+}
+
+void unpack_words(const uint64_t* header, const uint32_t* mask, const uint32_t* values, uint32_t* out,
+                  int64_t rows, int64_t wpr, int64_t tile_begin, int64_t tile_end) {
+  const int64_t tiles = (rows + kPackTileRows - 1) / kPackTileRows;
+  if (tile_begin < 0 || tile_end > tiles || tile_begin > tile_end)
+    throw std::runtime_error("unpack: tile range out of bounds");
+  const TileFn fn = tile_fn(current_variant());
+  const uint64_t total = header[0];
+  for (int64_t t = tile_begin; t < tile_end; ++t) {
+    const int64_t r0 = t * kPackTileRows, r1 = std::min<int64_t>(rows, r0 + kPackTileRows);
+    const int64_t e0 = r0 * wpr, n = (r1 - r0) * wpr;
+    const uint64_t off = header[1 + 2 * t], cnt = header[2 + 2 * t];
+    const uint32_t* m = mask + e0 / 32;
+    uint64_t bits = 0;
+    for (int64_t j = 0; j * 32 < n; ++j) bits += __builtin_popcount(m[j] & tail_bits(n - j * 32));
+    if (bits != cnt || off > total || cnt > total - off)
+      throw std::runtime_error("unpack: tile " + std::to_string(t) + ": header {" + std::to_string(off) + ", " +
+                               std::to_string(cnt) + "} against a mask of " + std::to_string(bits) + " words and " +
+                               std::to_string(total) + " values");
+    fn(m, values + off, values + total, out + e0, n);
+  }
+}
+
+
+void Job::wait() {
+  std::unique_lock<std::mutex> lk(mu_);
+  cv_.wait(lk, [&] { return pending_ == 0; });
+  if (error_) {
+    std::exception_ptr e = error_;
+    error_ = nullptr;
+    std::rethrow_exception(e);
+  }
+}
+
+bool Job::done() {
+  std::lock_guard<std::mutex> lk(mu_);
+  return pending_ == 0;
+}
+
+Pool::Pool(int threads) {
+  threads = std::max(1, threads);
+  workers_.reserve(threads);
+  for (int i = 0; i < threads; ++i) workers_.emplace_back([this] { worker(); });
+}
+
+Pool::~Pool() {
+  {
+    std::lock_guard<std::mutex> lk(mu_);
+    stop_ = true;
+  }
+  cv_.notify_all();
+  for (auto& w : workers_) w.join();
+}
+
+void Pool::worker() {
+  for (;;) {
+    std::function<void()> task;
+    {
+      std::unique_lock<std::mutex> lk(mu_);
+      cv_.wait(lk, [&] { return stop_ || !q_.empty(); });
+      if (q_.empty()) return;
+      task = std::move(q_.front());
+      q_.pop_front();
+    }
+    task();
+  }
+}
+
+std::shared_ptr<Job> Pool::post(int parts, std::function<void(int)> fn) {
+  auto job = std::make_shared<Job>();
+  if (parts <= 0) return job;
+  job->pending_ = parts;
+  auto shared_fn = std::make_shared<std::function<void(int)>>(std::move(fn));
+  {
+    std::lock_guard<std::mutex> lk(mu_);
+    for (int p = 0; p < parts; ++p)
+      q_.emplace_back([job, shared_fn, p] {
+        std::exception_ptr err;
+        try {
+          (*shared_fn)(p);
+        } catch (...) {
+          err = std::current_exception();
+        }
+        std::lock_guard<std::mutex> jl(job->mu_);
+        if (err && !job->error_) job->error_ = err;
+        if (--job->pending_ == 0) job->cv_.notify_all();
+      });
+  }
+  cv_.notify_all();
+  return job;
+}
+
+std::shared_ptr<Job> Pool::post_unpack(const void* packed, void* out, int64_t rows, int64_t wpr) {
+  const int64_t tiles = (rows + kPackTileRows - 1) / kPackTileRows;
+  const int parts = static_cast<int>(std::min<int64_t>(threads(), tiles));
+  return post(parts, [=](int p) {
+    unpack_buffer(packed, out, rows, wpr, tiles * p / parts, tiles * (p + 1) / parts);
+  });
+}
+
+int default_threads() {
+  if (const char* e = std::getenv("TFA_UNPACK_THREADS")) {
+    const int n = std::atoi(e);
+    if (n > 0) return std::min(n, 64);
+  }
+  int budget = 0;
+  if (const char* e = std::getenv("OMP_NUM_THREADS")) budget = std::atoi(e);
+#if defined(__linux__)
+  if (budget <= 0) {
+    cpu_set_t set;
+    CPU_ZERO(&set);
+    if (sched_getaffinity(0, sizeof(set), &set) == 0) budget = CPU_COUNT(&set);
+  }
+#endif
+  if (budget <= 0) budget = 4;
+  return std::max(1, std::min(12, budget - 2));
+}
+
+namespace {
+std::mutex g_pool_mu;
+std::unique_ptr<Pool> g_pool;
+}
+
+Pool& global_pool() {
+  std::lock_guard<std::mutex> lk(g_pool_mu);
+  if (!g_pool) g_pool = std::make_unique<Pool>(default_threads());
+  return *g_pool;
+}
+
+void shutdown_pool() {
+  std::unique_ptr<Pool> p;
+  {
+    std::lock_guard<std::mutex> lk(g_pool_mu);
+    p = std::move(g_pool);
+  }
+  p.reset();
+}
+
+}
+}
diff --git a/csrc/runtime/unpack.h b/csrc/runtime/unpack.h
--- /dev/null
+++ b/csrc/runtime/unpack.h
@@ -0,0 +1,76 @@
+#pragma once
+
+#include <condition_variable>
+#include <cstddef>
+#include <cstdint>
+#include <deque>
+#include <exception>
+#include <functional>
+#include <memory>
+#include <mutex>
+#include <thread>
+#include <vector>
+
+#include "../kernels/pack_layout.h"
+
+namespace tfa {
+namespace unpack {
+
+enum Variant : int { kAuto = -1, kScalar = 0, kAvx2 = 1, kAvx512 = 2 };
+
+bool variant_available(int v);
+void force_variant(int v);
+int current_variant();
+
+void unpack_words(const uint64_t* header, const uint32_t* mask, const uint32_t* values, uint32_t* out,
+                  int64_t rows, int64_t wpr, int64_t tile_begin, int64_t tile_end);
+
+inline void unpack_buffer(const void* packed, void* out, int64_t rows, int64_t wpr, int64_t tile_begin,
+                          int64_t tile_end) {
+  const PackLayout L = pack_layout(rows, wpr);
+  const char* p = static_cast<const char*>(packed);
+  unpack_words(reinterpret_cast<const uint64_t*>(p), reinterpret_cast<const uint32_t*>(p + L.mask_off),
+               reinterpret_cast<const uint32_t*>(p + L.values_off), static_cast<uint32_t*>(out), rows, wpr,
+               tile_begin, tile_end);
+}
+
+class Job {
+ public:
+  void wait();
+  bool done();
+
+ private:
+  friend class Pool;
+  std::mutex mu_;
+  std::condition_variable cv_;
+  int64_t pending_ = 0;
+  std::exception_ptr error_;
+};
+
+class Pool {
+ public:
+  explicit Pool(int threads);
+  ~Pool();
+  Pool(const Pool&) = delete;
+  Pool& operator=(const Pool&) = delete;
+  int threads() const { return static_cast<int>(workers_.size()); }
+
+  std::shared_ptr<Job> post(int parts, std::function<void(int)> fn);
+  std::shared_ptr<Job> post_unpack(const void* packed, void* out, int64_t rows, int64_t wpr);
+
+ private:
+  void worker();
+  std::mutex mu_;
+  std::condition_variable cv_;
+  std::deque<std::function<void()>> q_;
+  bool stop_ = false;
+  std::vector<std::thread> workers_;
+};
+
+int default_threads();
+
+Pool& global_pool();
+void shutdown_pool();
+
+}
+}
diff --git a/tensorframes_amd/config.py b/tensorframes_amd/config.py
--- a/tensorframes_amd/config.py
+++ b/tensorframes_amd/config.py
@@ -22,6 +22,7 @@
     chunk_bytes: int = dataclasses.field(default_factory=lambda: _env("TFA_CHUNK_BYTES", 128 << 20, int))
     min_pipeline_chunks: int = dataclasses.field(default_factory=lambda: _env("TFA_MIN_PIPELINE_CHUNKS", 16, int))
     pipeline_depth: int = dataclasses.field(default_factory=lambda: _env("TFA_PIPELINE_DEPTH", 3, int))
+    pack_outputs: bool = dataclasses.field(default_factory=lambda: _env("TFA_PACK_OUTPUTS", True, bool))
     min_chunked_rows: int = dataclasses.field(default_factory=lambda: _env("TFA_MIN_CHUNKED_ROWS", 65536, int))
     min_chunked_bytes: int = dataclasses.field(default_factory=lambda: _env("TFA_MIN_CHUNKED_BYTES", 32 << 20, int))
     stream_group_bytes: int = dataclasses.field(default_factory=lambda: _env("TFA_STREAM_GROUP_BYTES", 4 << 30, int))
@@ -74,6 +75,9 @@
         os.environ["TFA_DEBUG_SYNC"] = "1" if kw["debug_sync"] else "0"
         from ._native import _C
         _C.set_debug_sync(bool(kw["debug_sync"]))
+    if "pack_outputs" in kw:
+        from ._native import _C
+        _C.set_pack_outputs(bool(kw["pack_outputs"]))
     if "precision" in kw:
         apply_precision()
     if "pool_conv_fusion" in kw:
```

Measured after the change: 26.24 million rows/s, median of 6. 11.8% higher.
